# kocurvik/mdrp

Hardware: AMD Instinct MI355X
Metric: image-pairs/sec (2000 corrs, 10k RANSAC iters) (higher is better)
Workload: dtype f64

## Files before the change

### include/mdrp.h

```cpp
#ifndef MDRP_H
#define MDRP_H
#include <stddef.h>
#include <stdint.h>

#ifdef __cplusplus
extern "C" {
#endif

enum { MDRP_CALIB = 0, MDRP_SHARED_FOCAL = 1, MDRP_VARYING_FOCAL = 2,
       MDRP_RELPOSE_5PT = 3, MDRP_FUNDAMENTAL_7PT = 5,
       MDRP_SHARED_6PT = 4 };

enum {
    MDRP_OK = 0,
    MDRP_ERR_INVALID = 1,
    MDRP_ERR_HIP = 2,
    MDRP_ERR_NO_DEVICE = 3,
    MDRP_ERR_UNSUPPORTED = 4
};

enum {
    MDRP_MEM_HOST = 0,
    MDRP_MEM_DEVICE = 1
};

typedef struct {
    double q[4];
    double t[3];
    double scale, shift1, shift2;
    double f1, f2;
} mdrp_model;

typedef struct {
    uint64_t max_iterations;
    uint64_t min_iterations;
    double dyn_num_trials_mult;
    double success_prob;
    double max_reproj_error;
    double max_epipolar_error;
    uint64_t seed;
    int32_t monodepth_estimate_shift;
    float monodepth_weight_sampson;
    int32_t score_initial_model;
    int32_t progressive_sampling;
    uint64_t max_prosac_iterations;
    int32_t real_focal_check;
    int32_t reserved_;
} mdrp_ransac_opt;

typedef struct {
    uint64_t max_iterations;
    int32_t loss_type;
    double loss_scale;
    double gradient_tol;
    double step_tol;
    double initial_lambda;
    double min_lambda;
    double max_lambda;
} mdrp_bundle_opt;

typedef struct {
    int32_t model_id;
    int32_t pad_;
    double params[4];
} mdrp_camera;

typedef struct {
    mdrp_model model;
    uint64_t refinements, iterations, num_inliers;
    double inlier_ratio, model_score;
} mdrp_result;

typedef struct mdrp_handle mdrp_handle;

int mdrp_create_(int device, void *stream, mdrp_handle **out, int abi_version, int ransac_opt_bytes);
int mdrp_create_on_stream_(int device, void *stream, mdrp_handle **out, int abi_version, int ransac_opt_bytes);
#define mdrp_create(device, stream, out) mdrp_create_((device), (stream), (out), MDRP_ABI_VERSION, (int)sizeof(mdrp_ransac_opt))
#define mdrp_create_on_stream(device, stream, out) mdrp_create_on_stream_((device), (stream), (out), MDRP_ABI_VERSION, (int)sizeof(mdrp_ransac_opt))
void mdrp_destroy(mdrp_handle *h);
const char *mdrp_last_error(void);
const char *mdrp_version(void);
#define MDRP_ABI_VERSION 0x00000006
int mdrp_abi_version(void);
int mdrp_hip_build_version(void);
int mdrp_synchronize(mdrp_handle *h);


int mdrp_estimate_batch(mdrp_handle *h, int kind, int mem_space, const double *x1, const double *x2, const double *d1,
                        const double *d2, int batch, int n_max, const int32_t *n_per_pair, const mdrp_camera *cam1,
                        const mdrp_camera *cam2, const mdrp_ransac_opt *ropt, const mdrp_bundle_opt *bopt,
                        mdrp_result *out, uint8_t *inlier_mask);

int mdrp_estimate_batch_async(mdrp_handle *h, int kind, const double *x1_dev, const double *x2_dev, const double *d1_dev,
                              const double *d2_dev, int batch, int n_max, const int32_t *n_per_pair_host,
                              const mdrp_camera *cam1_host, const mdrp_camera *cam2_host, const mdrp_ransac_opt *ropt,
                              const mdrp_bundle_opt *bopt, uint8_t *inlier_mask_dev);
int mdrp_fetch_results(mdrp_handle *h, mdrp_result *out_host, int batch);
int mdrp_copy_results_device(mdrp_handle *h, void *dst_dev, int batch);

int mdrp_solver_batch(mdrp_handle *h, int solver, const double *x1h, const double *x2h, const double *d1,
                      const double *d2, int count, mdrp_model *out, int32_t *n_out);

int mdrp_classic_solver_batch(mdrp_handle *h, int kind, const double *x1h, const double *x2h, int count, mdrp_model *out,
                              int32_t *n_out);

int mdrp_score_models(mdrp_handle *h, int kind, int mem_space, const mdrp_model *models, int num_models,
                      const double *x1, const double *x2, int n, double sq_threshold, double *scores, int32_t *counts);

int mdrp_count_candidates(mdrp_handle *h, int kind, const mdrp_model *models, int num_models, const double *x1,
                          const double *x2, int n, double sq_threshold, int32_t *candidates);

int mdrp_bound_models(mdrp_handle *h, int kind, const mdrp_model *models, int num_models, const double *x1, const double *x2,
                      int n, double sq_threshold, double *score_lb, int32_t *count_ub);

#define MDRP_RETIRE_TWO_PHASE 1
#define MDRP_RETIRE_BOUND 2
#define MDRP_RETIRE_SWEEP_SCORE 0
#define MDRP_RETIRE_SWEEP_SPLIT 4
#define MDRP_RETIRE_SWEEP_WAVE 8
int mdrp_retire_models(mdrp_handle *h, int kind, const mdrp_model *models, int num_models, const double *x1, const double *x2,
                       int n, double sq_threshold, uint64_t rec_cnt, double rec_score, const uint64_t *cand_stat_in, int flags,
                       double *scores, int32_t *counts, int32_t *left_at, int32_t *info, uint64_t *cand_stat_out);

typedef struct {
    int32_t n, active;
    double sq_thr;
    uint64_t best_min_cnt;
    double best_min_score;
    uint64_t dyn_max_iter, iterations, refinements, num_inliers;
    double inlier_ratio, model_score;
    mdrp_model best;
} mdrp_replay_state;
typedef struct {
    uint32_t iter;
    int32_t k_ref;
    int32_t k_min;
    int32_t cnt_min;
    double score_min;
    int32_t cnt_ref;
    int32_t pad_;
} mdrp_replay_trigger;
typedef struct {
    int32_t mps, sample_sz, batch, n_chunks;
    uint64_t chunk_start;
    const int32_t *chunk_lens;
    const double *slot_score;
    const int32_t *slot_inl;
    const mdrp_model *models;
    const double *lo_score;
    const int32_t *lo_cnt;
    const mdrp_model *lo_models;
    const uint64_t *budgets;
    int32_t n_budgets, pad_;
    mdrp_replay_state *states;
    mdrp_replay_state *checkpoints;
    mdrp_replay_trigger *triggers;
    int32_t *n_triggers;
    uint64_t *scan_cnt;
    double *scan_score;
    int32_t *scan_inst;
    int32_t *lo_plan;
    int32_t *n_active;
    uint64_t *max_needed;
} mdrp_replay;
int mdrp_replay_slots(mdrp_handle *h, const mdrp_ransac_opt *ropt, mdrp_replay *io);

int mdrp_refine_models(mdrp_handle *h, int kind, mdrp_model *models, int count, const double *x1, const double *x2,
                       const double *d1, const double *d2, int n, double scale_reproj, double weight_sampson,
                       const mdrp_bundle_opt *opt, int estimate_shift, double *final_cost );

int mdrp_last_sweep_stats(mdrp_handle *h, double *sweep_ms, int64_t *launches, int64_t *evaluations);

typedef struct {
    double count_ms;
    int64_t count_launches;
    double sweep_ms;
    int64_t sweep_launches;
    int64_t evals_algorithmic;
    int64_t evals_mfma;
    int64_t evals_fp64;
    int64_t evals_bound;
    double lo_ms;
    int64_t lo_launches;
    double final_ms;
// ... 120 lines not shown
```

### mdrp_amd/_capi.py

```python
import ctypes as C
import os
import threading

import numpy as np

_HERE = os.path.dirname(os.path.abspath(__file__))
LIB_PATH = os.environ.get("MDRP_LIB") or os.path.join(_HERE, "libmdrp_hip.so")

CALIB, SHARED_FOCAL, VARYING_FOCAL = 0, 1, 2
RELPOSE_5PT, SHARED_6PT, FUNDAMENTAL_7PT = 3, 4, 5
MEM_HOST, MEM_DEVICE = 0, 1
SOLVER_P3P, SOLVER_SHIFT, SOLVER_SHARED, SOLVER_VARYING = 0, 1, 2, 3

EXPORTS = (
    "mdrp_create_", "mdrp_create_on_stream_", "mdrp_destroy", "mdrp_last_error", "mdrp_version", "mdrp_abi_version", "mdrp_hip_build_version", "mdrp_synchronize", "mdrp_estimate_batch",
    "mdrp_estimate_batch_async", "mdrp_fetch_results", "mdrp_copy_results_device", "mdrp_solver_batch", "mdrp_score_models", "mdrp_count_candidates", "mdrp_bound_models", "mdrp_refine_models",
    "mdrp_last_sweep_stats", "mdrp_last_stats", "mdrp_last_stats_sized", "mdrp_classic_solver_batch",
    "mdrp_gather_matches", "mdrp_estimate_matches_async",
    "mdrp_estimate_batch_budgets", "mdrp_estimate_batch_budgets_async", "mdrp_fetch_budget_results", "mdrp_copy_budget_results_device",
    "mdrp_refine_batch", "mdrp_refine_batch_async",
    "mdrp_gather_image_pairs", "mdrp_estimate_image_pairs_async",
    "mdrp_estimate_batch_prior", "mdrp_estimate_batch_prior_async",
    "mdrp_retire_models", "mdrp_replay_slots",
    "mdrp_estimate_batch_ranked", "mdrp_estimate_batch_ranked_async", "mdrp_prosac_samples", "mdrp_rank_scores",
    "mdrp_gather_matches_ranked", "mdrp_estimate_matches_ranked_async", "mdrp_gather_image_pairs_ranked", "mdrp_estimate_image_pairs_ranked_async",
)
RETIRE_TWO_PHASE, RETIRE_BOUND, RETIRE_SWEEP_SCORE, RETIRE_SWEEP_SPLIT, RETIRE_SWEEP_WAVE = 1, 2, 0, 4, 8
STAGE_LO, STAGE_INLIERS = 1, 2
MAX_BUDGETS = 16
F32, F64 = 0, 1
FILTERS = {"both_inf": 0, "finite": 1}


class Model(C.Structure):
    _fields_ = [("q", C.c_double * 4), ("t", C.c_double * 3), ("scale", C.c_double), ("shift1", C.c_double),
                ("shift2", C.c_double), ("f1", C.c_double), ("f2", C.c_double)]


class RansacOpt(C.Structure):
    _fields_ = [("max_iterations", C.c_uint64), ("min_iterations", C.c_uint64), ("dyn_num_trials_mult", C.c_double),
                ("success_prob", C.c_double), ("max_reproj_error", C.c_double), ("max_epipolar_error", C.c_double),
                ("seed", C.c_uint64), ("monodepth_estimate_shift", C.c_int32), ("monodepth_weight_sampson", C.c_float),
                ("score_initial_model", C.c_int32), ("progressive_sampling", C.c_int32), ("max_prosac_iterations", C.c_uint64),
                ("real_focal_check", C.c_int32), ("reserved_", C.c_int32)]


class BundleOpt(C.Structure):
    _fields_ = [("max_iterations", C.c_uint64), ("loss_type", C.c_int32), ("loss_scale", C.c_double),
                ("gradient_tol", C.c_double), ("step_tol", C.c_double), ("initial_lambda", C.c_double),
                ("min_lambda", C.c_double), ("max_lambda", C.c_double)]


class Camera(C.Structure):
    _fields_ = [("model_id", C.c_int32), ("pad_", C.c_int32), ("params", C.c_double * 4)]


class Stats(C.Structure):
    _fields_ = [("count_ms", C.c_double), ("count_launches", C.c_int64), ("sweep_ms", C.c_double), ("sweep_launches", C.c_int64),
                ("evals_algorithmic", C.c_int64), ("evals_mfma", C.c_int64), ("evals_fp64", C.c_int64), ("evals_bound", C.c_int64),
                ("lo_ms", C.c_double), ("lo_launches", C.c_int64), ("final_ms", C.c_double), ("final_launches", C.c_int64),
                ("bound_ms", C.c_double), ("bound_launches", C.c_int64), ("solve_ms", C.c_double), ("solve_launches", C.c_int64),
                ("lm_cost_evals", C.c_int64), ("lm_accum_evals", C.c_int64), ("final_cost_evals", C.c_int64), ("final_accum_evals", C.c_int64),
                ("fuse_gate_timeouts", C.c_int64), ("fuse_wait_timeouts", C.c_int64),
                ("first_chunk", C.c_int64)]


class Matches(C.Structure):
    _fields_ = [("kp1", C.c_void_p), ("kp2", C.c_void_p), ("kp_type", C.c_int32), ("k1", C.c_int32), ("k2", C.c_int32),
                ("matches", C.c_void_p), ("m_max", C.c_int32), ("depth1", C.c_void_p), ("depth2", C.c_void_p), ("depth_type", C.c_int32),
                ("h1", C.c_int32), ("w1", C.c_int32), ("h2", C.c_int32), ("w2", C.c_int32), ("center1", C.c_void_p), ("center2", C.c_void_p),
                ("filter", C.c_int32)]


class ImagePairs(C.Structure):
    _fields_ = [("kp", C.c_void_p), ("kp_type", C.c_int32), ("k_max", C.c_int32), ("kp_count", C.c_void_p), ("depth", C.c_void_p),
                ("depth_type", C.c_int32), ("h_max", C.c_int32), ("w_max", C.c_int32), ("size", C.c_void_p), ("center", C.c_void_p),
                ("n_images", C.c_int32), ("pairs", C.c_void_p), ("matches", C.c_void_p), ("m_max", C.c_int32), ("filter", C.c_int32)]


class Result(C.Structure):
    _fields_ = [("model", Model), ("refinements", C.c_uint64), ("iterations", C.c_uint64), ("num_inliers", C.c_uint64),
                ("inlier_ratio", C.c_double), ("model_score", C.c_double)]


MODEL_DTYPE = np.dtype([("q", "f8", 4), ("t", "f8", 3), ("scale", "f8"), ("shift1", "f8"), ("shift2", "f8"), ("f1", "f8"), ("f2", "f8")])
RESULT_DTYPE = np.dtype([("model", MODEL_DTYPE), ("refinements", "u8"), ("iterations", "u8"), ("num_inliers", "u8"),
                         ("inlier_ratio", "f8"), ("model_score", "f8")])
CAMERA_DTYPE = np.dtype([("model_id", "i4"), ("pad_", "i4"), ("params", "f8", 4)])
assert MODEL_DTYPE.itemsize == C.sizeof(Model) and RESULT_DTYPE.itemsize == C.sizeof(Result) and CAMERA_DTYPE.itemsize == C.sizeof(Camera)

REPLAY_STATE_DTYPE = np.dtype([("n", "i4"), ("active", "i4"), ("sq_thr", "f8"), ("best_min_cnt", "u8"), ("best_min_score", "f8"), ("dyn_max_iter", "u8"),
                               ("iterations", "u8"), ("refinements", "u8"), ("num_inliers", "u8"), ("inlier_ratio", "f8"), ("model_score", "f8"),
                               ("best", MODEL_DTYPE)])
REPLAY_TRIGGER_DTYPE = np.dtype([("iter", "u4"), ("k_ref", "i4"), ("k_min", "i4"), ("cnt_min", "i4"), ("score_min", "f8"), ("cnt_ref", "i4"), ("pad_", "i4")])


class Replay(C.Structure):
    _fields_ = [("mps", C.c_int32), ("sample_sz", C.c_int32), ("batch", C.c_int32), ("n_chunks", C.c_int32), ("chunk_start", C.c_uint64),
                ("chunk_lens", C.c_void_p), ("slot_score", C.c_void_p), ("slot_inl", C.c_void_p), ("models", C.c_void_p), ("lo_score", C.c_void_p),
                ("lo_cnt", C.c_void_p), ("lo_models", C.c_void_p), ("budgets", C.c_void_p), ("n_budgets", C.c_int32), ("pad_", C.c_int32),
# ... 12 lines not shown


def load_library():
    global _lib
    with _lib_lock:
        if _lib is not None:
            return _lib
        if not os.path.exists(LIB_PATH):
            raise MdrpError(f"{LIB_PATH} is not built (run __graft_entry__.build()); mdrp_amd has no CPU fallback")
        _ensure_hip_runtime()
        lib = C.CDLL(LIB_PATH)
        _check_hip_runtime_version(lib)
        vp, dp, ip = C.c_void_p, C.c_void_p, C.c_void_p
        lib.mdrp_last_error.restype = C.c_char_p
        lib.mdrp_version.restype = C.c_char_p
        abi = getattr(lib, "mdrp_abi_version", None)
        if abi is None or getattr(lib, "mdrp_create_", None) is None:
            raise MdrpError(f"{LIB_PATH} predates ABI {ABI_VERSION:#x} (no mdrp_abi_version / mdrp_create_): rebuild (mdrp_amd/build.py)")
        abi.restype = C.c_int
        if abi() != ABI_VERSION:
            raise MdrpError(f"{LIB_PATH} speaks ABI {abi():#x}, this binding {ABI_VERSION:#x}: rebuild (mdrp_amd/build.py)")
        lib.mdrp_create_.argtypes = [C.c_int, vp, C.POINTER(vp), C.c_int, C.c_int]
        lib.mdrp_create_on_stream_.argtypes = [C.c_int, vp, C.POINTER(vp), C.c_int, C.c_int]
        lib.mdrp_destroy.argtypes = [vp]
        lib.mdrp_destroy.restype = None
        lib.mdrp_synchronize.argtypes = [vp]
        lib.mdrp_estimate_batch.argtypes = [vp, C.c_int, C.c_int, dp, dp, dp, dp, C.c_int, C.c_int, ip, vp, vp,
                                            C.POINTER(RansacOpt), C.POINTER(BundleOpt), vp, vp]
        lib.mdrp_estimate_batch_async.argtypes = [vp, C.c_int, dp, dp, dp, dp, C.c_int, C.c_int, ip, vp, vp,
                                                  C.POINTER(RansacOpt), C.POINTER(BundleOpt), vp]
        lib.mdrp_fetch_results.argtypes = [vp, vp, C.c_int]
        lib.mdrp_copy_results_device.argtypes = [vp, vp, C.c_int]
        lib.mdrp_solver_batch.argtypes = [vp, C.c_int, dp, dp, dp, dp, C.c_int, vp, vp]
        lib.mdrp_score_models.argtypes = [vp, C.c_int, C.c_int, vp, C.c_int, dp, dp, C.c_int, C.c_double, vp, vp]
        lib.mdrp_count_candidates.argtypes = [vp, C.c_int, vp, C.c_int, dp, dp, C.c_int, C.c_double, vp]
        lib.mdrp_bound_models.argtypes = [vp, C.c_int, vp, C.c_int, dp, dp, C.c_int, C.c_double, vp, vp]
        lib.mdrp_refine_models.argtypes = [vp, C.c_int, vp, C.c_int, dp, dp, dp, dp, C.c_int, C.c_double, C.c_double,
                                           C.POINTER(BundleOpt), C.c_int, vp]
        lib.mdrp_last_sweep_stats.argtypes = [vp, C.POINTER(C.c_double), C.POINTER(C.c_int64), C.POINTER(C.c_int64)]
        lib.mdrp_last_stats.argtypes = [vp, C.POINTER(Stats)]
        lib.mdrp_last_stats_sized.argtypes = [vp, C.POINTER(Stats), C.c_size_t]
        lib.mdrp_classic_solver_batch.argtypes = [vp, C.c_int, dp, dp, C.c_int, vp, vp]
        lib.mdrp_gather_matches.argtypes = [vp, C.POINTER(Matches), C.c_int, dp, dp, dp, dp, ip, ip]
        lib.mdrp_estimate_matches_async.argtypes = [vp, C.c_int, C.POINTER(Matches), C.c_int, vp, vp, C.POINTER(RansacOpt), C.POINTER(BundleOpt), vp, ip]
        if hasattr(lib, "mdrp_estimate_batch_budgets"):
            lib.mdrp_estimate_batch_budgets.argtypes = [vp, C.c_int, C.c_int, dp, dp, dp, dp, C.c_int, C.c_int, ip, vp, vp,
                                                        C.POINTER(RansacOpt), C.POINTER(BundleOpt), vp, C.c_int, vp, vp]
            lib.mdrp_estimate_batch_budgets_async.argtypes = [vp, C.c_int, dp, dp, dp, dp, C.c_int, C.c_int, ip, vp, vp,
                                                              C.POINTER(RansacOpt), C.POINTER(BundleOpt), vp, C.c_int, vp]
            lib.mdrp_fetch_budget_results.argtypes = [vp, vp, C.c_int, C.c_int]
            lib.mdrp_copy_budget_results_device.argtypes = [vp, vp, C.c_int, C.c_int]
        if hasattr(lib, "mdrp_refine_batch"):
            lib.mdrp_refine_batch.argtypes = [vp, C.c_int, C.c_int, dp, dp, dp, dp, C.c_int, C.c_int, ip, vp, vp,
                                              C.POINTER(RansacOpt), C.POINTER(BundleOpt), vp, C.c_int, vp, vp, dp, ip]
            lib.mdrp_refine_batch_async.argtypes = [vp, C.c_int, dp, dp, dp, dp, C.c_int, C.c_int, ip, vp, vp,
                                                    C.POINTER(RansacOpt), C.POINTER(BundleOpt), vp, C.c_int, vp, dp, ip]
        if hasattr(lib, "mdrp_gather_image_pairs"):
            lib.mdrp_gather_image_pairs.argtypes = [vp, C.POINTER(ImagePairs), C.c_int, dp, dp, dp, dp, ip, ip]
            lib.mdrp_estimate_image_pairs_async.argtypes = [vp, C.c_int, C.POINTER(ImagePairs), C.c_int, vp, vp, C.POINTER(RansacOpt), C.POINTER(BundleOpt), vp, ip]
        if hasattr(lib, "mdrp_estimate_batch_ranked"):
            lib.mdrp_estimate_batch_ranked.argtypes = [vp, C.c_int, C.c_int, dp, dp, dp, dp, dp, C.c_int, C.c_int, ip, vp, vp,
                                                       C.POINTER(RansacOpt), C.POINTER(BundleOpt), vp, vp]
            lib.mdrp_estimate_batch_ranked_async.argtypes = [vp, C.c_int, dp, dp, dp, dp, dp, C.c_int, C.c_int, ip, vp, vp,
                                                             C.POINTER(RansacOpt), C.POINTER(BundleOpt), vp]
            lib.mdrp_prosac_samples.argtypes = [vp, C.c_uint64, C.c_int, C.c_uint64, ip, C.c_int, vp]
            lib.mdrp_rank_scores.argtypes = [vp, C.c_int, vp, C.c_int, C.c_int, ip, vp]
        if hasattr(lib, "mdrp_gather_matches_ranked"):
            lib.mdrp_gather_matches_ranked.argtypes = [vp, C.POINTER(Matches), vp, C.c_int, C.c_int, dp, dp, dp, dp, ip, ip]
            lib.mdrp_estimate_matches_ranked_async.argtypes = [vp, C.c_int, C.POINTER(Matches), vp, C.c_int, C.c_int, vp, vp, C.POINTER(RansacOpt),
                                                               C.POINTER(BundleOpt), vp, ip]
            lib.mdrp_gather_image_pairs_ranked.argtypes = [vp, C.POINTER(ImagePairs), vp, C.c_int, C.c_int, dp, dp, dp, dp, ip, ip]
            lib.mdrp_estimate_image_pairs_ranked_async.argtypes = [vp, C.c_int, C.POINTER(ImagePairs), vp, C.c_int, C.c_int, vp, vp, C.POINTER(RansacOpt),
                                                                   C.POINTER(BundleOpt), vp, ip]
        if hasattr(lib, "mdrp_estimate_batch_prior"):
            lib.mdrp_estimate_batch_prior.argtypes = [vp, C.c_int, C.c_int, dp, dp, dp, dp, C.c_int, C.c_int, ip, vp, vp,
                                                      C.POINTER(RansacOpt), C.POINTER(BundleOpt), vp, vp, vp]
            lib.mdrp_estimate_batch_prior_async.argtypes = [vp, C.c_int, dp, dp, dp, dp, C.c_int, C.c_int, ip, vp, vp,
                                                            C.POINTER(RansacOpt), C.POINTER(BundleOpt), vp, vp]
        if hasattr(lib, "mdrp_retire_models"):
            lib.mdrp_retire_models.argtypes = [vp, C.c_int, vp, C.c_int, dp, dp, C.c_int, C.c_double, C.c_uint64, C.c_double, vp, C.c_int,
                                               vp, vp, vp, vp, vp]
        if hasattr(lib, "mdrp_replay_slots"):
            lib.mdrp_replay_slots.argtypes = [vp, C.POINTER(RansacOpt), C.POINTER(Replay)]
        _lib = lib
        return lib


ABI_VERSION = 0x00000006
ERR_UNSUPPORTED = 4


def _check(lib, rc):
    if rc == ERR_UNSUPPORTED:
        raise NotImplementedError(f"mdrp: {lib.mdrp_last_error().decode(errors='replace')} (DESIGN.md 9)")
    if rc != 0:
        raise MdrpError(f"mdrp error {rc}: {lib.mdrp_last_error().decode(errors='replace')}")


def _ptr(a):
    return None if a is None else C.c_void_p(a.ctypes.data)


def ransac_opt_from_dict(d=None):
    d = d or {}
    return RansacOpt(int(d.get("max_iterations", 100000)), int(d.get("min_iterations", 1000)),
                     float(d.get("dyn_num_trials_mult", 3.0)), float(d.get("success_prob", 0.9999)),
                     float(d.get("max_reproj_error", 12.0)), float(d.get("max_epipolar_error", 1.0)),
                     int(d.get("seed", 0)), int(bool(d.get("monodepth_estimate_shift", False))),
                     float(d.get("monodepth_weight_sampson", 1.0)), int(bool(d.get("score_initial_model", False))),
                     int(bool(d.get("progressive_sampling", False))), int(d.get("max_prosac_iterations", 100000)),
                     int(bool(d.get("real_focal_check", False))), 0)


LOSS_TYPES = {"TRIVIAL": 0, "TRUNCATED": 1, "HUBER": 2, "CAUCHY": 3, "TRUNCATED_CAUCHY": 4, "TRUNCATED_LE_ZACH": 5}


def bundle_opt_from_dict(d=None):
    d = d or {}
    lt = d.get("loss_type", "CAUCHY")
    if isinstance(lt, str):
        if lt.upper() not in LOSS_TYPES:
            raise ValueError(f"unknown loss_type {lt!r}")
        lt = LOSS_TYPES[lt.upper()]
    return BundleOpt(int(d.get("max_iterations", 100)), int(lt), float(d.get("loss_scale", 1.0)),
                     float(d.get("gradient_tol", 1e-10)), float(d.get("step_tol", 1e-8)), float(d.get("initial_lambda", 1e-3)),
                     float(d.get("min_lambda", 1e-10)), float(d.get("max_lambda", 1e10)))


def budget_list(budgets, ransac_opt=None):
    try:
        ks = [int(k) for k in budgets]
        exact = all(k == b for k, b in zip(ks, budgets))
    except (TypeError, ValueError):
        raise ValueError("budgets must be a sequence of integers") from None
    if not ks:
        raise ValueError("budgets: an empty list")
    if not exact:
        raise ValueError("budgets must be integers")
    if len(ks) > MAX_BUDGETS:
        raise ValueError(f"budgets: more than {MAX_BUDGETS}")
    if ks[0] < 1 or any(b <= a for a, b in zip(ks, ks[1:])):
        raise ValueError("budgets must be >= 1 and strictly increasing")
    ro = dict(ransac_opt or {})
    if "max_iterations" in ro and int(ro["max_iterations"]) != ks[-1]:
        raise ValueError(f"ransac_opt['max_iterations'] = {ro['max_iterations']} differs from the last budget {ks[-1]}")
    ro["max_iterations"] = ks[-1]
    return np.asarray(ks, dtype=np.uint64), ro


def library_version():
    return load_library().mdrp_version().decode()


def library_source_hash():
    v = library_version()
    return v.split("MDRP_SRC_HASH=", 1)[1][:16] if "MDRP_SRC_HASH=" in v else None


_hip_runtime = None
hip_versions = None


def _check_hip_runtime_version(lib):
    import warnings
    try:
        lib.mdrp_hip_build_version.restype = C.c_int
        built = int(lib.mdrp_hip_build_version())
        v = C.c_int(0)
        rt = _hip_runtime.hipRuntimeGetVersion
        rt.argtypes = [C.POINTER(C.c_int)]
        if rt(C.byref(v)) != 0:
            return
    except (AttributeError, OSError):
        return
    have = int(v.value)
    if have // 10_000_000 != built // 10_000_000:
        raise MdrpError(f"libmdrp_hip.so was built against HIP {built // 10_000_000}.{built // 100_000 % 100} but the process's HIP runtime "
                        f"({getattr(_hip_runtime, '_name', '?')}) is {have // 10_000_000}.{have // 100_000 % 100}: set MDRP_HIP_RUNTIME to a "
                        "matching libamdhip64.so or rebuild (mdrp_amd/build.py)")
    global hip_versions
    hip_versions = {"built": built, "runtime": have}
    if have // 100_000 != built // 100_000 and os.environ.get("MDRP_DEBUG"):
        warnings.warn(f"mdrp: HIP runtime {have // 10_000_000}.{have // 100_000 % 100} in this process, library built against "
                      f"{built // 10_000_000}.{built // 100_000 % 100} (same major: continuing)", RuntimeWarning, stacklevel=3)


def _ensure_hip_runtime():
    global _hip_runtime
    if _hip_runtime is not None:
        return _hip_runtime
    import sys
    cands = []
    if os.environ.get("MDRP_HIP_RUNTIME"):
        cands.append(os.environ["MDRP_HIP_RUNTIME"])
    try:
        torch = sys.modules.get("torch")
        if torch is not None:
            tdir = os.path.dirname(torch.__file__)
        else:
            import importlib.util
            spec = importlib.util.find_spec("torch")
            tdir = list(spec.submodule_search_locations)[0] if spec is not None and spec.submodule_search_locations else None
        if tdir and os.path.exists(os.path.join(tdir, "lib", "libamdhip64.so")):
            cands.append(os.path.join(tdir, "lib", "libamdhip64.so"))
    except Exception:
        pass
    import glob
    rocm = os.environ.get("ROCM_PATH", "/opt/rocm")
    def _soname_version(path):
        tail = os.path.basename(path).split(".so.", 1)[-1]
        return tuple(int(x) for x in tail.split(".") if x.isdigit())
    cands += sorted(glob.glob(os.path.join(rocm, "lib", "libamdhip64.so.*")), key=_soname_version, reverse=True) + ["libamdhip64.so", os.path.join(rocm, "lib", "libamdhip64.so")]
    errs = []
    for c in cands:
        try:
            _hip_runtime = C.CDLL(c, mode=C.RTLD_GLOBAL)
            return _hip_runtime
        except OSError as e:
            errs.append(f"{c}: {e}")
    raise MdrpError("no HIP runtime (libamdhip64) could be loaded: " + "; ".join(errs))


class Handle:

    def __init__(self, device=0, stream=None):
        self._lib = load_library()
        h = C.c_void_p()
        if stream is None:
            _check(self._lib, self._lib.mdrp_create_(int(device), None, C.byref(h), ABI_VERSION, C.sizeof(RansacOpt)))
        else:
# ... 475 lines not shown
```

### mdrp_amd/build.py

```python
import hashlib
import os
import re
import shutil
import subprocess

HERE = os.path.dirname(os.path.abspath(__file__))
SRC = os.path.join(HERE, "csrc", "mdrp_capi.hip")
SRC_TU = os.path.join(HERE, "csrc", "mdrp_tu.hip")
TU_GROUPS = (1, 2, 3, 4, 5)
DEPS = [SRC, SRC_TU, os.path.join(HERE, "csrc", "mdrp_kernels.h"), os.path.join(HERE, "csrc", "mdrp_math.h"),
        os.path.join(HERE, "csrc", "mdrp_classic.h"), os.path.join(HERE, "csrc", "mdrp_classic_math.h"),
        os.path.join(HERE, "csrc", "mdrp_logtab.h"), os.path.join(HERE, "csrc", "mdrp_instances.h"),
        os.path.join(HERE, "csrc", "mdrp_frontend.h"), os.path.join(HERE, "csrc", "mdrp_schedule.h"),
        os.path.join(HERE, "csrc", "mdrp_from_model.h"), os.path.join(HERE, "csrc", "mdrp_prior.h"), os.path.join(HERE, "csrc", "mdrp_prosac.h"),
        os.path.join(HERE, "..", "include", "mdrp.h")]
OUT = os.path.join(HERE, "libmdrp_hip.so")
_MARK = b"MDRP_SRC_HASH="
FLAGS = ["-O3", "-std=c++17", "--offload-arch=gfx950", "-fPIC", "-shared", "-ffp-contract=fast", "-no-hip-rt"]


def hipcc():
    for c in (shutil.which("hipcc"), "/opt/rocm/bin/hipcc"):
        if c and os.path.exists(c):
            return c
    raise RuntimeError("hipcc not found")


def source_hash():
    h = hashlib.sha256()
    h.update(" ".join(FLAGS).encode())
    for d in DEPS:
        h.update(os.path.basename(d).encode() + b"\0")
        with open(d, "rb") as f:
            h.update(f.read())
    return h.hexdigest()[:16]


def built_hash(path=OUT):
    try:
        with open(path, "rb") as f:
            m = re.search(_MARK + rb"([0-9a-f]{16})", f.read())
        return m.group(1).decode() if m else None
    except OSError:
        return None


def up_to_date():
    return built_hash() == source_hash()


def build(force=False, verbose=False, defines=(), out=OUT, extra_flags=(), single=None):
    if not force and not defines and not extra_flags and out == OUT and up_to_date():
        return out
    if single is None:
        single = bool(defines) or bool(extra_flags)
    common = [*FLAGS, *extra_flags, f'-DMDRP_SRC_HASH="{source_hash()}"', *[f"-D{d}" for d in defines]]
    if verbose:
        common.insert(0, "-Rpass-analysis=kernel-resource-usage")
    if single:
        subprocess.check_call([hipcc(), *common, SRC, "-o", out + ".tmp"])
        os.replace(out + ".tmp", out)
        return out
    import tempfile
    from concurrent.futures import ThreadPoolExecutor
    cflags = [f for f in common if f != "-shared"]
    with tempfile.TemporaryDirectory(prefix="mdrp_build_") as tmp:
        jobs = [([hipcc(), *cflags, "-DMDRP_SPLIT_TU", "-c", SRC, "-o", os.path.join(tmp, "capi.o")], os.path.join(tmp, "capi.o"))]
        for g in TU_GROUPS:
            obj = os.path.join(tmp, f"tu{g}.o")
            jobs.append(([hipcc(), *cflags, f"-DMDRP_TU={g}", "-c", SRC_TU, "-o", obj], obj))

        def run(job):
            r = subprocess.run(job[0], capture_output=True, text=True)
            return job, r
        with ThreadPoolExecutor(max_workers=len(jobs)) as pool:
            results = list(pool.map(run, jobs))
        for (cmd, obj), r in results:
            if verbose or r.returncode != 0:
                import sys
                sys.stderr.write(r.stderr)
            if r.returncode != 0:
                raise subprocess.CalledProcessError(r.returncode, cmd, r.stdout, r.stderr)
        subprocess.check_call([hipcc(), "--offload-arch=gfx950", "-shared", "-fPIC", "-no-hip-rt", *[o for _, o in jobs], "-o", out + ".tmp"])
    os.replace(out + ".tmp", out)
    return out


if __name__ == "__main__":
    print(build(force=True, verbose=True))
```

### mdrp_amd/csrc/mdrp_capi.hip

```cpp
#include "../../include/mdrp.h"
#include "mdrp_kernels.h"
#include "mdrp_classic.h"
#include "mdrp_frontend.h"
#include "mdrp_schedule.h"
#include "mdrp_from_model.h"
#include "mdrp_prior.h"
#include "mdrp_prosac.h"
#ifdef MDRP_SPLIT_TU
#define MDRP_INST extern
#include "mdrp_instances.h"
namespace mdrp {
MDRP_INSTANCES_FINAL_64
MDRP_INSTANCES_FINAL_256
MDRP_INSTANCES_CLASSIC
MDRP_INSTANCES_FROM_MODEL
MDRP_INSTANCES_PRIOR
}
#endif

#include <algorithm>
#include <cmath>
#include <cstdio>
#include <cstdlib>
#include <cstddef>
// ... 29 lines not shown
struct DevBuf {
    void *p = nullptr;
    size_t cap = 0;
    DevBuf() = default;
    DevBuf(const DevBuf &) = delete;
    DevBuf &operator=(const DevBuf &) = delete;
    ~DevBuf() { release(); }
    int ensure(size_t bytes) {
        if (bytes <= cap) return MDRP_OK;
        if (p) { (void)hipFree(p); p = nullptr; cap = 0; }
        size_t want = bytes + bytes / 8 + 256;
        hipError_t e = hipMalloc(&p, want);
        if (e != hipSuccess) { g_err = std::string("hipMalloc failed: ") + hipGetErrorString(e); p = nullptr; return MDRP_ERR_HIP; }
        cap = want;
        return MDRP_OK;
    }
    void release() { if (p) (void)hipFree(p); p = nullptr; cap = 0; }
    template <typename T> T *as() const { return reinterpret_cast<T *>(p); }
};

template <typename T, auto Destroy> struct Owned {
    T v = nullptr;
    Owned() = default;
    Owned(Owned &&o) noexcept : v(o.v) { o.v = nullptr; }
    Owned(const Owned &) = delete;
    Owned &operator=(const Owned &) = delete;
    ~Owned() { reset(); }
    void reset() { if (v) (void)Destroy(v); v = nullptr; }
    operator T() const { return v; }
    T operator->() const { return v; }
};
using Stream = Owned<hipStream_t, hipStreamDestroy>;
using Event = Owned<hipEvent_t, hipEventDestroy>;
template <typename T> using Pinned = Owned<T *, hipHostFree>;

struct Progress {
    int32_t n_active, pad_;
    unsigned long long max_needed;
    unsigned long long evals;
    unsigned long long evals_mfma;
    unsigned long long evals_sweep;
    unsigned long long evals_bound;
    int32_t wish_sum, wish_pairs;
};
struct Counters {
    int32_t unused_[2];
    Progress progress;
    int32_t lo_head[16];
    int32_t xcd_head[8 * LO_XCD_STRIDE];
};
static_assert(offsetof(Counters, progress) == 2 * sizeof(int32_t) && offsetof(Counters, lo_head) == 16 * sizeof(int32_t) &&
              offsetof(Counters, xcd_head) == 32 * sizeof(int32_t) && sizeof(Counters) == 640, "counter block layout");
static_assert(offsetof(Progress, evals_mfma) == offsetof(Progress, evals) + sizeof(unsigned long long), "k_count adds to stats[0] and stats[1]");
static_assert(offsetof(Progress, wish_pairs) == offsetof(Progress, wish_sum) + sizeof(int32_t), "RunParams::inl_stat is [2]");
constexpr size_t LM_STATS_BYTES = 6 * sizeof(unsigned long long);

struct DeviceGuard {
    int prev = -1;
    bool ok = true;
    explicit DeviceGuard(int device) {
        if (hipGetDevice(&prev) != hipSuccess) prev = -1;
        if (prev != device) ok = hipSetDevice(device) == hipSuccess;
    }
    ~DeviceGuard() {
        int cur = -1;
        if (prev >= 0 && hipGetDevice(&cur) == hipSuccess && cur != prev) (void)hipSetDevice(prev);
    }
};

}

struct mdrp_handle {
    std::mutex mu;
    int device = 0;
    hipStream_t stream = nullptr;
    Stream own_stream;
    Stream aux_stream;
    Stream aux_stream2;
    Stream copy_stream;
    Event ev_copied, ev_prepped, ev_solved6;
    DevBuf fuse;
    Event ev_lo, ev_tables, ev_sampled[2], ev_solved[sched::NC_MAX], ev_scanned[sched::NC_MAX];
    int num_cu = 256;
    DevBuf pts, dep, st;
    DevBuf params;
    Pinned<unsigned char> params_host;
    size_t params_host_cap = 0;
    DevBuf models, slot_score, slot_inl, triggers, work_pair, counters, results, mask, plan;
    DevBuf samples[2], tags[2], model_count[2];
    DevBuf tags_sorted[2];
    DevBuf tags_v, surv_count;
    DevBuf cand_stat;
    DevBuf und_count;
    DevBuf rfrag;
    DevBuf cplan;
    DevBuf surv2_count;
    DevBuf lo_mask;
    DevBuf red5;
    DevBuf lm_stats;
    Pinned<unsigned long long> lm_stats_host;
    int64_t fuse_gate_timeouts = 0, fuse_wait_timeouts = 0;
    int64_t first_chunk = 0;
    double seen_wish[3] = {-1.0, -1.0, -1.0};
    Pinned<int32_t> wish_host; Event ev_wish;
    int wish_kind = -1;
    bool fuse_disabled = false;
    int fuse_retry_in = 0;
    int fuse_backoff = 64;
    DevBuf ckpt, ck_list, bresults, bmask;
    int last_budgets = 0;
    DevBuf in_x1, in_x2, in_d1, in_d2;
    DevBuf fm_models, fm_init;
    DevBuf pr_x1, pr_x2, pr_d1, pr_d2, pr_order, pr_mask, pr_scores, pr_nper, pr_tab;
    DevBuf fe_key;
    DevBuf fe_x1, fe_x2, fe_d1, fe_d2, fe_slot, fe_n;
    Pinned<int32_t> fe_n_host;
    size_t fe_n_host_cap = 0;
    DevBuf unit_a, unit_b, unit_c, unit_d, unit_e, unit_f;
    Pinned<Progress> progress_host;
    std::vector<std::pair<Event, Event>> ev_pool;
    std::vector<int> ev_what;
    size_t ev_used = 0;
    double sweep_ms = 0.0, count_ms = 0.0;
    double kind_ms[6] = {0, 0, 0, 0, 0, 0};
    int64_t kind_launches[6] = {0, 0, 0, 0, 0, 0};
    int64_t lm_cost_evals = 0, lm_accum_evals = 0, fin_cost_evals = 0, fin_accum_evals = 0;
    int64_t count_launches = 0;
    int64_t sweep_launches = 0, sweep_evals = 0, mfma_evals = 0, fp64_evals = 0, bound_evals = 0;
    int last_batch = 0;
};

namespace {

#define MDRP_LM_DISPATCH_T(KERNEL, T, kind, shift, grid, smem, stream, ...)                                          \
    do {                                                                                                             \
        if ((kind) == 0 && (shift)) hipLaunchKernelGGL((KERNEL<0, true, T>), grid, dim3(T), smem, stream, __VA_ARGS__);  \
        else if ((kind) == 0) hipLaunchKernelGGL((KERNEL<0, false, T>), grid, dim3(T), smem, stream, __VA_ARGS__);       \
        else if ((kind) == 1) hipLaunchKernelGGL((KERNEL<1, false, T>), grid, dim3(T), smem, stream, __VA_ARGS__);       \
        else hipLaunchKernelGGL((KERNEL<2, false, T>), grid, dim3(T), smem, stream, __VA_ARGS__);                        \
    } while (0)
#define MDRP_LM_DISPATCH(KERNEL, threads, kind, shift, grid, smem, stream, ...)                                      \
    do {                                                                                                             \
        if ((threads) == 64) MDRP_LM_DISPATCH_T(KERNEL, 64, kind, shift, grid, smem, stream, __VA_ARGS__);           \
        else MDRP_LM_DISPATCH_T(KERNEL, 256, kind, shift, grid, smem, stream, __VA_ARGS__);                          \
    } while (0)

#define MDRP_FINAL_DISPATCH_L(T, FL, kind, shift, grid, smem, stream, ...)                                                  \
    do {                                                                                                                   \
        if ((kind) == 0 && (shift)) hipLaunchKernelGGL((k_final<0, true, T, FL>), grid, dim3(T), smem, stream, __VA_ARGS__);  \
        else if ((kind) == 0) hipLaunchKernelGGL((k_final<0, false, T, FL>), grid, dim3(T), smem, stream, __VA_ARGS__);       \
        else if ((kind) == 1) hipLaunchKernelGGL((k_final<1, false, T, FL>), grid, dim3(T), smem, stream, __VA_ARGS__);       \
        else hipLaunchKernelGGL((k_final<2, false, T, FL>), grid, dim3(T), smem, stream, __VA_ARGS__);                        \
    } while (0)
#define MDRP_FINAL_DISPATCH_T(T, floss, kind, shift, grid, smem, stream, ...)                                               \
    do {                                                                                                                   \
        switch (floss) {                                                                                                   \
        case 1: MDRP_FINAL_DISPATCH_L(T, 1, kind, shift, grid, smem, stream, __VA_ARGS__); break;                          \
        case 2: MDRP_FINAL_DISPATCH_L(T, 2, kind, shift, grid, smem, stream, __VA_ARGS__); break;                          \
        case 3: MDRP_FINAL_DISPATCH_L(T, 3, kind, shift, grid, smem, stream, __VA_ARGS__); break;                          \
        case 4: MDRP_FINAL_DISPATCH_L(T, 4, kind, shift, grid, smem, stream, __VA_ARGS__); break;                          \
        case 5: MDRP_FINAL_DISPATCH_L(T, 5, kind, shift, grid, smem, stream, __VA_ARGS__); break;                          \
        default: MDRP_FINAL_DISPATCH_L(T, 0, kind, shift, grid, smem, stream, __VA_ARGS__); break;  \
        }                                                                                                                  \
    } while (0)
#define MDRP_FINAL_DISPATCH(threads, floss, kind, shift, grid, smem, stream, ...)                                           \
    do {                                                                                                                   \
// ... 105 lines not shown
}
constexpr int HOST_SLICE_PAIRS = 256;

struct PassIn {
    int kind;
    const double *x1, *x2, *d1, *d2;
    int batch, n_max;
    const int32_t *n_host;
    const mdrp_camera *cam1, *cam2;
    const mdrp_ransac_opt *ro;
    const mdrp_bundle_opt *bo;
    int chunk_cap;
    uint8_t *mask_dev;
    ResultDev *results_dev;
    const HostSrc *host;
    int batch_call;
    const BudgetOut *bud;
    const Model *priors;
    const uint64_t *prosac;
};

struct ProsacTab { uint64_t *k; const uint64_t *off; const uint32_t *sub; };
void launch_samples_prosac(hipStream_t st, int threads, int n_tables, const int32_t *d_table_n, uint64_t *d_table_state, const ProsacTab &tab,
                           uint64_t max_prosac, int len, uint32_t *smp) {
    hipLaunchKernelGGL(k_samples_prosac, dim3(n_tables), dim3(threads), 0, st, n_tables, d_table_n, d_table_state, tab.k, tab.off, tab.sub,
                       prosac::prosac_samples(max_prosac), len, smp);
}
int prosac_tables(mdrp_handle *h, hipStream_t s, const int32_t *tab_n, int n_tables, uint64_t max_prosac, uint64_t count, ProsacTab &tab) {
    std::vector<uint64_t> head(2 * (size_t)n_tables + 1, 0);
    std::vector<uint32_t> sub;
    for (int t = 0; t < n_tables; ++t) {
        const std::vector<uint32_t> one = prosac::subset_schedule((uint64_t)std::max(tab_n[t], 0), max_prosac, count, true);
        head[n_tables + t] = sub.size();
        sub.insert(sub.end(), one.begin(), one.end());
    }
    head[2 * (size_t)n_tables] = sub.size();
    const size_t hb = sizeof(uint64_t) * head.size(), sb = sizeof(uint32_t) * sub.size();
    if (int rc = h->pr_tab.ensure(hb + sb + 16)) return rc;
    unsigned char *d = h->pr_tab.as<unsigned char>();
    HIPCHK(hipMemcpyAsync(d, head.data(), hb, hipMemcpyHostToDevice, s));
    if (sb) HIPCHK(hipMemcpyAsync(d + hb, sub.data(), sb, hipMemcpyHostToDevice, s));
    tab.k = reinterpret_cast<uint64_t *>(d); tab.off = tab.k + n_tables; tab.sub = reinterpret_cast<const uint32_t *>(d + hb);
    return MDRP_OK;
}

int launch_scan(hipStream_t s, int mps, int pairs, const RunParams &r, PairState *st, const double *slot_score, const int32_t *slot_inl, Trigger *trig,
                int trig_cap, const int32_t *model_count, unsigned long long *scan_stats) {
#define MDRP_SCAN(M, I)                                                                                                                            \
    do {                                                                                                                                           \
        hipLaunchKernelGGL((k_scan<M, I>), dim3(pairs), dim3(64), 0, s, r, st, slot_score, slot_inl, trig, trig_cap, model_count, scan_stats);      \
        return 10 * M + I;                                                                                                                         \
    } while (0)
    if (mps == 16) MDRP_SCAN(16, 1);
    if (mps == 12) MDRP_SCAN(12, 1);
    if (r.chunk_len >= 1024) MDRP_SCAN(4, 4);
    MDRP_SCAN(4, 1);
#undef MDRP_SCAN
}

struct ChunkView {
    int c, p0, pc;
    bool first_of_run;
    RunParams r;
    PairState *st;
    double *pts, *dep, *slot_score;
    Model *models;
    int32_t *slot_inl, *model_count, *surv1, *surv2, *und_count;
    uint32_t *samples, *tags, *tags_sorted, *tags_sorted_other, *tags_v;
    unsigned long long *cand_stat;
    uint4 *rfrag;
    Trigger *trig;
};
struct Survivors { const uint32_t *tags; const int32_t *count; };

struct Pass : PassIn {
    mdrp_handle *const h;
    const hipStream_t s;
    const int est_shift;
    const bool classic;
    const int mps, ssz;
    const bool lo_overlap = env_int("MDRP_LO_OVERLAP", 1) != 0;
    const bool use_bound = env_int("MDRP_BOUND", 1) != 0;
    const bool score_split = env_int("MDRP_SCORE_SPLIT", 1) != 0;
    const int lo_threads = env_int("MDRP_LO_THREADS", sched::lo_lanes(batch_call, n_max));
    const int final_threads = env_int("MDRP_FINAL_THREADS", sched::final_lanes(batch_call));
    const int samp_threads = env_int("MDRP_SAMPLE_THREADS", ssz == 3 ? SAMP_THREADS : (ssz == 5 ? 512 : 256));
    const int lo_blocks = h->num_cu * (lo_threads == 64 ? 8 : 2);
    const int mask_index = lm_mask_index_on(n_max);
    const int clm_list_stride = lm_list_stride(n_max);
    const size_t clm_list_bytes = (size_t)2 * clm_list_stride * sizeof(uint16_t);
    const bool fuse_env = !bud && env_int("MDRP_FUSE_TAIL", ((kind == MDRP_CALIB && est_shift) || h->fuse_disabled) ? 0 : 1) != 0;
    const int n_bud = bud ? bud->n : 0;
    const int trig_cap = chunk_cap;
    const size_t groups_max = ((size_t)n_max + 15) / 16;

    std::vector<int32_t> table_of, tab_n;
    int n_tables = 0;
    uint64_t certain = 0;
    sched::Lead lead;
    PassScratch sz;
    RunParams rp;
    unsigned char *pd = nullptr;
    uint64_t *d_table_state = nullptr;
    CamDev *d_cams1 = nullptr, *d_cams2 = nullptr;
    int32_t *d_table_n = nullptr, *d_table_of = nullptr, *d_nper = nullptr;
    Counters *cnt = nullptr;
    uint64_t it0 = 0;
    sched::Layout lay;
    bool piped = false, fuse_tail = false, presampled[2] = {false, false};
    hipStream_t aux = nullptr, aux2 = nullptr;
    int32_t *fz_ctl = nullptr, *fz_done = nullptr, *fz_fin = nullptr, *fz_ready = nullptr;
    bool final_done = false;
    ProsacTab ptab{nullptr, nullptr, nullptr};

    Pass(mdrp_handle *h_, const PassIn &in)
        : PassIn(in), h(h_), s(h_->stream), est_shift((kind == MDRP_CALIB && ro->monodepth_estimate_shift) ? 1 : 0), classic(kind >= MDRP_RELPOSE_5PT),
          mps(sched::model_slots(kind)), ssz(sched::sample_size(kind)) {}

    int plan_and_allocate() {
        sched::group_tables(n_host, batch, table_of, tab_n);
        n_tables = (int)tab_n.size();
        certain = sched::certain_iterations(ro->max_iterations, ro->min_iterations);
        const bool chunks_set = sched::parse_chunks(getenv("MDRP_CHUNKS"), lead);
        if (h->wish_kind >= 0 && hipEventQuery(h->ev_wish) == hipSuccess) {
            if (h->wish_host[1] > 0) h->seen_wish[h->wish_kind] = (double)h->wish_host[0] / (double)h->wish_host[1];
            h->wish_kind = -1;
        }
        if (!chunks_set) lead = sched::default_lead(kind, certain, kind <= MDRP_VARYING_FOCAL ? h->seen_wish[kind] : -1.0);
        sz = pass_scratch(h, kind, batch, n_max, n_tables, chunk_cap, lead.first(), n_bud);
        for (const auto &b : sz.bufs) {
            if (int rc = b.first->ensure(b.second)) return rc;
            if (b.first == &h->params && h->params_host_cap < sz.params) {
                h->params_host.reset(); h->params_host_cap = 0;
                HIPCHK(hipHostMalloc((void **)&h->params_host.v, sz.params + sz.params / 2, hipHostMallocDefault));
                h->params_host_cap = sz.params + sz.params / 2;
            }
        }
        pd = h->params.as<unsigned char>();
        d_table_state = reinterpret_cast<uint64_t *>(pd);
        d_cams1 = reinterpret_cast<CamDev *>(pd + sz.off_cam1); d_cams2 = reinterpret_cast<CamDev *>(pd + sz.off_cam2);
        d_table_n = reinterpret_cast<int32_t *>(pd + sz.off_tn); d_table_of = reinterpret_cast<int32_t *>(pd + sz.off_tof);
        d_nper = reinterpret_cast<int32_t *>(pd + sz.off_nper);
        cnt = h->counters.as<Counters>();
        return MDRP_OK;
    }

    int upload_params() {
        unsigned char *ph = h->params_host;
        const std::vector<uint64_t> tab_state(n_tables, ro->seed);
        std::memcpy(ph, tab_state.data(), sizeof(uint64_t) * n_tables);
        const bool cams = kind == MDRP_CALIB || kind == MDRP_RELPOSE_5PT || kind == MDRP_SHARED_6PT;
        if (cams) { std::memcpy(ph + sz.off_cam1, cam1, sizeof(CamDev) * batch); std::memcpy(ph + sz.off_cam2, cam2 ? cam2 : cam1, sizeof(CamDev) * batch); }
        else std::memset(ph + sz.off_cam1, 0, 2 * sizeof(CamDev) * (size_t)batch);
        std::memcpy(ph + sz.off_tn, tab_n.data(), sizeof(int32_t) * n_tables);
        std::memcpy(ph + sz.off_tof, table_of.data(), sizeof(int32_t) * batch);
        std::memcpy(ph + sz.off_nper, n_host, sizeof(int32_t) * batch);
        if (bud) std::memcpy(ph + sz.off_bud, bud->budgets, sizeof(uint64_t) * n_bud);
        HIPCHK(hipMemcpyAsync(pd, ph, sz.params, hipMemcpyHostToDevice, s));
        if (prosac) { if (int rc = prosac_tables(h, s, tab_n.data(), n_tables, *prosac, ro->max_iterations, ptab)) return rc; }

        std::memset(&rp, 0, sizeof rp);
        rp.kind = kind; rp.solver = solver_for(kind, est_shift); rp.est_shift = est_shift;
        rp.score_initial = ro->score_initial_model ? 1 : 0;
        rp.batch = batch; rp.n_max = n_max;
        rp.max_iterations = ro->max_iterations; rp.min_iterations = ro->min_iterations;
        rp.dyn_mult = ro->dyn_num_trials_mult; rp.log_prob_missing = std::log(1.0 - ro->success_prob);
// ... 1 lines not shown
        rp.final_max_it = (int)std::min<uint64_t>(bo->max_iterations, 1u << 30); rp.final_loss = bo->loss_type;
        rp.grad_tol = bo->gradient_tol; rp.step_tol = bo->step_tol; rp.lambda0 = bo->initial_lambda;
        rp.lambda_min = bo->min_lambda; rp.lambda_max = bo->max_lambda;
        rp.chunk_len = chunk_cap; rp.chunk_off = 0; rp.slot_stride = chunk_cap * mps; rp.super_len = chunk_cap; rp.chunk_start = 0;
        rp.mps = mps; rp.sample_sz = ssz;
        return MDRP_OK;
    }

    void prep(int p0, int pc, hipStream_t st_) {
        const size_t o2 = (size_t)2 * p0 * n_max, o1 = (size_t)p0 * n_max;
        double *pts_p = h->pts.as<double>() + o1 * PT_STRIDE;
        uint4 *rfrag_p = h->rfrag.as<uint4>() + (size_t)p0 * groups_max * 64;
        if (classic)
            hipLaunchKernelGGL(kc_prep, dim3(pc), dim3(256), 0, st_, rp, x1 + o2, x2 + o2, d_nper + p0, d_table_of + p0, d_cams1 + p0, d_cams2 + p0,
                               ro->max_epipolar_error, bo->loss_scale, pts_p, h->st.as<PairState>() + p0, rfrag_p);
        else
            hipLaunchKernelGGL(k_prep, dim3(pc), dim3(256), 0, st_, rp, x1 + o2, x2 + o2, d1 + o1, d2 + o1, d_nper + p0, d_table_of + p0, d_cams1 + p0, d_cams2 + p0,
                               ro->max_epipolar_error, ro->max_reproj_error, bo->loss_scale, pts_p, h->dep.as<double>() + 2 * o1, h->st.as<PairState>() + p0, rfrag_p);
    }

    void prior() {
#define MDRP_PRIOR_LAUNCH(K, S)                                                                                                                  \
    hipLaunchKernelGGL((k_prior<K, S>), dim3(batch), dim3(PRIOR_THREADS), lm_list_bytes(n_max), s, rp, h->st.as<PairState>(),                     \
                       (const double *)h->pts.as<double>(), (const double *)h->dep.as<double>(), priors, lm_list_stride(n_max),                  \
                       h->lm_stats.as<unsigned long long>())
        if (kind == MDRP_CALIB && est_shift) MDRP_PRIOR_LAUNCH(0, true);
        else if (kind == MDRP_CALIB) MDRP_PRIOR_LAUNCH(0, false);
        else if (kind == MDRP_SHARED_FOCAL) MDRP_PRIOR_LAUNCH(1, false);
        else MDRP_PRIOR_LAUNCH(2, false);
#undef MDRP_PRIOR_LAUNCH
    }

    int begin_super_chunk(uint64_t max_needed) {
        lay = sched::super_chunk_layout(it0, certain, chunk_cap, lead, max_needed, ro->max_iterations);
        if (it0 == 0) h->first_chunk = (int64_t)lay.lens[0];
        rp.chunk_start = it0; rp.super_len = (int)lay.super_len;
        HIPCHK(hipMemsetAsync(h->counters.p, 0, sizeof(Counters), s));
        if (it0 == 0) HIPCHK(hipMemsetAsync(h->cand_stat.p, 0, sizeof(unsigned long long) * 2 * batch, s));
        piped = lay.n_chunks > 1 && lo_overlap;
        fuse_tail = fuse_env && piped && it0 + lay.super_len >= ro->max_iterations;
        if (fuse_tail) {
            if (int rc = h->fuse.ensure(sz.fuse)) return rc;
            fz_ctl = h->fuse.as<int32_t>(); fz_done = fz_ctl + 16; fz_fin = fz_done + batch; fz_ready = fz_fin + batch;
        }
        aux = piped ? h->aux_stream : s; aux2 = piped ? h->aux_stream2 : s;
        presampled[0] = presampled[1] = false;
        return MDRP_OK;
    }

    void samples(hipStream_t st_, int len_, uint32_t *smp_) {
        if (prosac) launch_samples_prosac(st_, samp_threads, n_tables, d_table_n, d_table_state, ptab, *prosac, len_, smp_);
        else if (ssz == 6) hipLaunchKernelGGL(kc_samples<6>, dim3(n_tables), dim3(samp_threads), 0, st_, n_tables, d_table_n, d_table_state, len_, smp_);
        else if (ssz == 5) hipLaunchKernelGGL(kc_samples<5>, dim3(n_tables), dim3(samp_threads), 0, st_, n_tables, d_table_n, d_table_state, len_, smp_);
        else if (ssz == 7) hipLaunchKernelGGL(kc_samples<7>, dim3(n_tables), dim3(samp_threads), 0, st_, n_tables, d_table_n, d_table_state, len_, smp_);
        else hipLaunchKernelGGL(k_samples, dim3(n_tables), dim3(samp_threads), 0, st_, n_tables, d_table_n, d_table_state, len_, smp_);
    }
    int presample() {
        HIPCHK(hipStreamWaitEvent(aux2, h->ev_tables, 0));
        for (int c = 0; c < 2 && c < lay.n_chunks; ++c) {
            samples(aux2, (int)lay.lens[c], h->samples[c & 1].as<uint32_t>());
            HIPCHK(hipEventRecord(h->ev_sampled[c], aux2));
            presampled[c] = true;
        }
        return MDRP_OK;
    }

    ChunkView view(int c, int p0, int pc) const {
        ChunkView v;
        const bool odd = c & 1;
        const size_t so = (size_t)p0 * rp.slot_stride, o1 = (size_t)p0 * n_max, q = (size_t)p0;
        v.c = c; v.p0 = p0; v.pc = pc; v.first_of_run = it0 == 0 && c == 0;
        v.r = rp; v.r.chunk_len = (int)lay.lens[c]; v.r.chunk_off = lay.offs[c]; v.r.batch = pc;
        v.st = h->st.as<PairState>() + q; v.pts = h->pts.as<double>() + o1 * PT_STRIDE; v.dep = classic ? nullptr : h->dep.as<double>() + o1 * 2;
        v.models = h->models.as<Model>() + so; v.slot_score = h->slot_score.as<double>() + so; v.slot_inl = h->slot_inl.as<int32_t>() + so;
        v.samples = h->samples[odd].as<uint32_t>(); v.tags = h->tags[odd].as<uint32_t>() + so; v.tags_v = h->tags_v.as<uint32_t>() + so;
        v.tags_sorted = h->tags_sorted[odd].as<uint32_t>() + so; v.tags_sorted_other = h->tags_sorted[!odd].as<uint32_t>() + so;
        v.model_count = h->model_count[odd].as<int32_t>() + 2 * q; v.und_count = h->und_count.as<int32_t>() + 2 * q;
        v.surv1 = h->surv_count.as<int32_t>() + q; v.surv2 = h->surv2_count.as<int32_t>() + q;
        v.cand_stat = h->cand_stat.as<unsigned long long>() + 2 * q;
        v.rfrag = h->rfrag.as<uint4>() + q * groups_max * 64; v.trig = h->triggers.as<Trigger>() + q * trig_cap;
        return v;
    }

    int solve(const ChunkView &v, hipStream_t st_) {
        const RunParams &r = v.r;
        const int pc = v.pc;
        HIPCHK(hipMemsetAsync(v.model_count, 0, sizeof(int32_t) * 2 * pc, st_));
        if (v.c < 2 && presampled[v.c]) HIPCHK(hipStreamWaitEvent(st_, h->ev_sampled[v.c], 0));
        else samples(st_, r.chunk_len, v.samples);
        hipEvent_t v0, v1;
        if (int rc = get_events(h, &v0, &v1, 5)) return rc;
        HIPCHK(hipEventRecord(v0, st_));
        struct Stop { hipEvent_t e; hipStream_t s; ~Stop() { (void)hipEventRecord(e, s); } } stop_{v1, st_};
        if (classic) {
            const dim3 sgrid((r.chunk_len + 63) / 64, pc);
            if (kind == MDRP_SHARED_6PT)
                hipLaunchKernelGGL(kc_solve<CLASSIC_SHARED>, sgrid, dim3(64), 0, st_, r, v.st, v.samples, v.pts, v.models, v.slot_inl, v.tags, v.model_count);
            else if (kind == MDRP_RELPOSE_5PT) {
                const bool first_region = v.c == 0 && lay.n_chunks > 1;
                if (first_region && (size_t)sgrid.x > sz.red5_first_blocks) { g_err = "5-point first chunk longer than its Reduce5 region"; return MDRP_ERR_INVALID; }
                double *red5 = h->red5.as<double>() + ((first_region ? (size_t)batch * sz.red5_blocks : 0) + (size_t)v.p0 * sgrid.x) * RED5_STRIDE * 64;
                hipLaunchKernelGGL(kc_solve5_null, sgrid, dim3(64), SOLVE5N_LDS_BYTES, st_, r, v.st, v.samples, v.pts, red5);
                hipLaunchKernelGGL(kc_solve5_reduce, sgrid, dim3(64), SOLVE5_LDS_BYTES, st_, r, v.st, red5);
                hipLaunchKernelGGL(kc_solve5_roots, sgrid, dim3(64), SOLVE5B_LDS_BYTES, st_, r, v.st, v.samples, v.pts, red5, v.models, v.slot_inl, v.tags, v.model_count);
            }
            else
                hipLaunchKernelGGL(kc_solve<CLASSIC_FUND>, sgrid, dim3(64), SOLVE7_LDS_BYTES, st_, r, v.st, v.samples, v.pts, v.models, v.slot_inl, v.tags, v.model_count);
            return MDRP_OK;
        }
#define MDRP_SOLVE_LAUNCH(S)                                                                                                   \
    hipLaunchKernelGGL(k_solve<S>, dim3((r.chunk_len + solve_threads(S) - 1) / solve_threads(S), pc), dim3(solve_threads(S)), 0, st_, r, v.st, v.samples, v.pts, v.dep, v.models, v.slot_inl, v.tags, v.model_count, 0, r.chunk_len)
        switch (r.solver) {
        case SOLVER_P3P: MDRP_SOLVE_LAUNCH(SOLVER_P3P); break;
        case SOLVER_SHIFT: MDRP_SOLVE_LAUNCH(SOLVER_SHIFT); break;
        case SOLVER_SHARED: MDRP_SOLVE_LAUNCH(SOLVER_SHARED); break;
        default: MDRP_SOLVE_LAUNCH(SOLVER_VARYING); break;
        }
#undef MDRP_SOLVE_LAUNCH
        return MDRP_OK;
    }

    int count(const ChunkView &v) {
        unsigned long long *cstats = &cnt->progress.evals;
        hipEvent_t c0, c1;
        if (int rc = get_events(h, &c0, &c1, 1)) return rc;
        const bool two_phase = !v.first_of_run;
        uint32_t *tags_u = v.tags_sorted;
        int32_t *und_part = reinterpret_cast<int32_t *>(v.tags_sorted_other), *cplan = h->cplan.as<int32_t>();
        hipLaunchKernelGGL(k_count_plan, dim3(1), dim3(PLAN_THREADS), 0, s, v.pc, v.st, v.model_count, 2, CNT_WG_MODELS, cplan,
                           v.surv1, (const int32_t *)nullptr, two_phase ? v.und_count : (int32_t *)nullptr);
        const dim3 cgrid((unsigned)v.pc * (unsigned)((v.r.chunk_len * mps + CNT_WG_MODELS - 1) / CNT_WG_MODELS));
        HIPCHK(hipEventRecord(c0, s));
        MDRP_SWEEP_DISPATCH(k_count, kind, cgrid, dim3(CNT_THREADS), 0, s, v.r, v.st, v.rfrag, v.models,
                            v.tags, v.model_count, cplan, v.tags_v, v.surv1, cstats, (int32_t *)nullptr, (const int32_t *)nullptr,
                            1, tags_u, und_part, v.und_count, (const int32_t *)nullptr, v.cand_stat);
        if (two_phase) {
            hipLaunchKernelGGL(k_count_plan, dim3(1), dim3(PLAN_THREADS), 0, s, v.pc, v.st, v.und_count, 2, CNT_WG_MODELS, cplan,
                               (int32_t *)nullptr, (const int32_t *)nullptr, (int32_t *)nullptr);
            MDRP_SWEEP_DISPATCH(k_count, kind, cgrid, dim3(CNT_THREADS), 0, s, v.r, v.st, v.rfrag, v.models,
                                tags_u, v.und_count, cplan, v.tags_v, v.surv1, cstats, (int32_t *)nullptr, (const int32_t *)nullptr,
                                2, (uint32_t *)nullptr, (int32_t *)nullptr, (int32_t *)nullptr, und_part, v.cand_stat);
            h->count_launches++;
        }
        HIPCHK(hipEventRecord(c1, s));
        h->count_launches++;
        return MDRP_OK;
    }

    int bound(const ChunkView &v, Survivors &sv) {
        sv = Survivors{v.tags_v, v.surv1};
        if (!(use_bound && batch_call > 16 && !v.first_of_run)) return MDRP_OK;
        hipLaunchKernelGGL(k_count_plan, dim3(1), dim3(PLAN_THREADS), 0, s, v.pc, v.st, v.surv1, 1, BND_THREADS, h->cplan.as<int32_t>(), v.surv2, (const int32_t *)nullptr);
        const dim3 bgrid((unsigned)v.pc * (unsigned)((v.r.chunk_len * mps + BND_THREADS - 1) / BND_THREADS));
        unsigned long long *bstats = &cnt->progress.evals_bound;
        hipEvent_t b0, b1;
        if (int rc = get_events(h, &b0, &b1, 4)) return rc;
        HIPCHK(hipEventRecord(b0, s));
        MDRP_SWEEP_DISPATCH(k_bound, kind, bgrid, dim3(BND_THREADS), 0, s, v.r, v.st, v.pts, v.models, v.tags_v, v.surv1, h->cplan.as<int32_t>(), v.tags, v.surv2, bstats);
        HIPCHK(hipEventRecord(b1, s));
        sv = Survivors{v.tags, v.surv2};
        return MDRP_OK;
    }

    int score(const ChunkView &v, const Survivors &sv, hipEvent_t e0, hipEvent_t e1) {
        const bool wave = batch_call <= SCORE_WAVE_MAX_PAIRS, split = !wave && score_split && !v.first_of_run;
        const int models = v.r.chunk_len * mps;
        int32_t *plan = h->plan.as<int32_t>(), *totals = plan + 2 * (size_t)batch + 2;
        if (wave) hipLaunchKernelGGL(k_count_plan, dim3(1), dim3(PLAN_THREADS), 0, s, v.pc, v.st, sv.count, 1, SCW_THREADS / 64, plan, (int32_t *)nullptr, (const int32_t *)nullptr, (int32_t *)nullptr);
        hipLaunchKernelGGL(k_sort_tags, dim3(v.pc), dim3(256), 0, s, v.r, v.st, v.model_count, sv.count, sv.tags, v.tags_sorted);
        if (!wave) hipLaunchKernelGGL(k_plan, dim3(1), dim3(PLAN_THREADS), 0, s, v.pc, v.model_count, plan, totals, split ? SPLIT_HYP : SCORE_THREADS);
        HIPCHK(hipEventRecord(e0, s));
        const long long capped = (long long)h->num_cu * 32;
        if (wave) {
            const long long ub = (long long)v.pc * ((models + SCW_THREADS / 64 - 1) / (SCW_THREADS / 64));
            MDRP_SWEEP_DISPATCH(k_score_w, kind, dim3((unsigned)std::min(ub, capped)), dim3(SCW_THREADS), 0, s, v.r, v.st, v.pts, v.models, v.tags_sorted, v.model_count,
                                v.slot_score, v.slot_inl, plan);
        } else if (split) {
            const long long ub = (long long)v.pc * ((models + SPLIT_HYP - 1) / SPLIT_HYP + 1);
            MDRP_SWEEP_DISPATCH(k_score_split, kind, dim3((unsigned)std::min(ub, capped)), dim3(SPLIT_THREADS), 0, s, v.r, v.st, v.pts, v.models, v.tags_sorted, v.model_count,
                                v.slot_score, v.slot_inl, plan, totals);
        } else {
            const dim3 grid((unsigned)v.pc * (unsigned)((models + SCORE_THREADS - 1) / SCORE_THREADS));
            MDRP_SWEEP_DISPATCH(k_score, kind, grid, dim3(SCORE_THREADS), SCORE_TILE_BYTES, s, v.r, v.st, v.pts, v.models, v.tags_sorted, v.model_count,
                                v.slot_score, v.slot_inl, plan, totals);
        }
        HIPCHK(hipEventRecord(e1, s));
        h->sweep_launches++;
        return MDRP_OK;
    }

    void scan(const ChunkView &v) {
        (void)launch_scan(s, mps, v.pc, v.r, v.st, v.slot_score, v.slot_inl, v.trig, trig_cap, v.model_count, &cnt->progress.evals_sweep);
    }

    int sweep(const ChunkView &v) {
        hipEvent_t e0, e1;
        Survivors sv;
        int rc;
        if ((rc = get_events(h, &e0, &e1, 0)) || (rc = count(v)) || (rc = bound(v, sv)) || (rc = score(v, sv, e0, e1))) return rc;
        scan(v);
        return MDRP_OK;
    }

    int first_chunk_of(int q0, int qc) {
        const ChunkView v = view(0, q0, qc);
        int rc;
        if (kind != MDRP_SHARED_6PT) { if ((rc = solve(v, s))) return rc; }
        else {
            if ((rc = solve(v, aux))) return rc;
            HIPCHK(hipEventRecord(h->ev_solved6, aux));
            HIPCHK(hipStreamWaitEvent(s, h->ev_solved6, 0));
        }
        return sweep(v);
    }
    int host_front(bool &solved1, int &swept0) {
        int rc;
        const bool sliced = piped && lay.n_chunks >= 2 && batch >= 2 * HOST_SLICE_PAIRS;
        const int sl = sliced ? HOST_SLICE_PAIRS : batch;
        for (int p0 = 0; p0 < batch; p0 += sl) {
            const int pc = std::min(sl, batch - p0);
            const size_t o2 = (size_t)2 * p0 * n_max, o1 = (size_t)p0 * n_max, n2 = sizeof(double) * 2 * (size_t)pc * n_max, n1 = sizeof(double) * (size_t)pc * n_max;
            hipStream_t cs = sliced ? h->copy_stream : s;
            HIPCHK(hipMemcpyAsync(const_cast<double *>(x1) + o2, host->x1 + o2, n2, hipMemcpyHostToDevice, cs));
            HIPCHK(hipMemcpyAsync(const_cast<double *>(x2) + o2, host->x2 + o2, n2, hipMemcpyHostToDevice, cs));
            if (host->d1 && host->d2) {
                HIPCHK(hipMemcpyAsync(const_cast<double *>(d1) + o1, host->d1 + o1, n1, hipMemcpyHostToDevice, cs));
                HIPCHK(hipMemcpyAsync(const_cast<double *>(d2) + o1, host->d2 + o1, n1, hipMemcpyHostToDevice, cs));
            }
            if (!sliced) { prep(p0, pc, s); break; }
            HIPCHK(hipEventRecord(h->ev_copied, cs)); HIPCHK(hipStreamWaitEvent(aux, h->ev_copied, 0));
            if (p0 == 0) HIPCHK(hipStreamWaitEvent(aux, h->ev_tables, 0));
            prep(p0, pc, aux);
            HIPCHK(hipEventRecord(h->ev_prepped, aux));
            if ((rc = solve(view(1, p0, pc), aux))) return rc;
            const bool last = p0 + sl >= batch, last_but_one = !last && p0 + 2 * sl >= batch;
            if (last_but_one || last) HIPCHK(hipStreamWaitEvent(s, h->ev_prepped, 0));
            if (last_but_one) { swept0 = p0 + pc; if ((rc = first_chunk_of(0, swept0))) return rc; }
            if (last) { if ((rc = first_chunk_of(swept0, batch - swept0))) return rc; swept0 = batch; }
        }
        if (sliced) { HIPCHK(hipEventRecord(h->ev_solved[1], aux)); solved1 = true; }
        return MDRP_OK;
    }

    int lo(int c) {
        int32_t *lo_plan = h->work_pair.as<int32_t>();
        hipLaunchKernelGGL(k_lo_plan, dim3(1), dim3(PLAN_THREADS), 0, s, batch, h->st.as<PairState>(), (const int32_t *)nullptr, lo_plan);
        if (fuse_tail) {
            HIPCHK(hipMemsetAsync(fz_ctl, 0, 64 + 2 * sizeof(int32_t) * (size_t)batch, s));
            HIPCHK(hipMemsetAsync(fz_ready, 0xFF, sizeof(int32_t) * (size_t)batch, s));
        }
        if (piped) { HIPCHK(hipEventRecord(h->ev_scanned[c], s)); HIPCHK(hipStreamWaitEvent(aux2, h->ev_scanned[c], 0)); }
        const FuseTail fz = fuse_tail ? FuseTail{fz_done, fz_ready, fz_ctl, h->st.as<PairState>()} : FuseTail{nullptr, nullptr, nullptr, nullptr};
        unsigned long long *lm_stats = h->lm_stats.as<unsigned long long>();
        int32_t *xheads = cnt->xcd_head;
        hipEvent_t l0, l1;
        if (int rc = get_events(h, &l0, &l1, 2)) return rc;
        HIPCHK(hipEventRecord(l0, aux2));
        if (classic)
            MDRP_CLASSIC_LM_DISPATCH(kc_lo, lo_threads, kind, dim3(lo_blocks), clm_list_bytes, aux2, rp, h->st.as<PairState>(), h->pts.as<double>(),
                                     h->models.as<Model>(), h->triggers.as<Trigger>(), trig_cap, lo_plan, cnt->lo_head, xheads,
                                     h->lo_mask.as<uint8_t>(), clm_list_stride, fz);
        else
            MDRP_LM_DISPATCH(k_lo, lo_threads, kind, est_shift, dim3(lo_blocks), lm_list_bytes(n_max), aux2, rp,
                             h->st.as<PairState>(), h->pts.as<double>(), h->dep.as<double>(), h->models.as<Model>(), h->triggers.as<Trigger>(),
                             trig_cap, lo_plan, cnt->lo_head, xheads, lm_list_stride(n_max), lm_stats, fz);
        HIPCHK(hipEventRecord(l1, aux2));
        return MDRP_OK;
    }

    void final_of(const RunParams &rf, int problems, PairState *st_f, uint8_t *mask_f, ResultDev *results_f, const int32_t *ready, int32_t *fin_done,
                  unsigned long long ticks, unsigned long long *timeouts) {
        if (classic)
            MDRP_CLASSIC_LM_DISPATCH(kc_final, final_threads, kind, dim3(problems), clm_list_bytes, s, rf, st_f, h->pts.as<double>(), mask_f, results_f,
                                     ready, fin_done, ticks, timeouts, clm_list_stride);
        else
            MDRP_FINAL_DISPATCH(final_threads, rf.final_loss, kind, est_shift, dim3(problems), (mask_index ? lm_final_list_bytes(n_max) : lm_list_bytes(n_max)), s, rf,
                                st_f, h->pts.as<double>(), h->dep.as<double>(), mask_f, results_f, lm_list_stride(n_max), mask_index,
                                h->lm_stats.as<unsigned long long>() + 2, ready, fin_done, ticks, timeouts);
    }
    void final_pairs(const int32_t *ready, int32_t *fin_done, unsigned long long ticks, unsigned long long *timeouts) {
        final_of(rp, batch, h->st.as<PairState>(), mask_dev, results_dev, ready, fin_done, ticks, timeouts);
    }
// ... 193 lines not shown
int finish_timing(mdrp_handle *h) {
    if (h->lm_stats.p) HIPCHK(hipMemcpyAsync(h->lm_stats_host, h->lm_stats.p, LM_STATS_BYTES, hipMemcpyDeviceToHost, h->stream));
    HIPCHK(hipStreamSynchronize(h->stream));
    h->lm_cost_evals = (int64_t)h->lm_stats_host[0]; h->lm_accum_evals = (int64_t)h->lm_stats_host[1];
    h->fin_cost_evals = (int64_t)h->lm_stats_host[2]; h->fin_accum_evals = (int64_t)h->lm_stats_host[3];
    h->fuse_gate_timeouts = (int64_t)h->lm_stats_host[4]; h->fuse_wait_timeouts = (int64_t)h->lm_stats_host[5];
    if (!(h->fuse_gate_timeouts || h->fuse_wait_timeouts) && !h->fuse_disabled) h->fuse_backoff = 64;
    if ((h->fuse_gate_timeouts || h->fuse_wait_timeouts) && !h->fuse_disabled) {
        h->fuse_disabled = true;
        h->fuse_retry_in = h->fuse_backoff;
        h->fuse_backoff = std::min(h->fuse_backoff * 2, 16384);
        if (!getenv("MDRP_QUIET"))
            fprintf(stderr, "[mdrp] fused tail: %lld gate / %lld final-refinement waits timed out (kernels of two streams did not overlap: "
                            "profiler or serialised dispatch?); this handle runs unfused for its next %d calls\n",
                    (long long)h->fuse_gate_timeouts, (long long)h->fuse_wait_timeouts, h->fuse_retry_in);
    }
    for (int k = 0; k < 6; ++k) { h->kind_ms[k] = 0; h->kind_launches[k] = 0; }
    for (size_t i = 0; i < h->ev_used; ++i) {
        float t = 0;
        HIPCHK(hipEventElapsedTime(&t, h->ev_pool[i].first, h->ev_pool[i].second));
        const int k = std::min(std::max(h->ev_what[i], 0), 5);
        h->kind_ms[k] += t; h->kind_launches[k]++;
    }
    h->sweep_ms = h->kind_ms[0]; h->count_ms = h->kind_ms[1];
    return MDRP_OK;
}

}

#define MDRP_ENTER(h)                                                                      \
    std::lock_guard<std::mutex> lock_((h)->mu);                                            \
    DeviceGuard guard_((h)->device);                                                       \
    if (!guard_.ok) { g_err = "hipSetDevice failed"; return MDRP_ERR_HIP; }

#ifndef MDRP_SRC_HASH
#define MDRP_SRC_HASH "unknown"
#endif

static int create_handle(int device, hipStream_t stream, bool own_stream, mdrp_handle **out);

extern "C" {

const char *mdrp_last_error(void) { return g_err.c_str(); }
int mdrp_abi_version(void) { return MDRP_ABI_VERSION; }
const char *mdrp_version(void) { return "mdrp-hip 0.6 (gfx950) MDRP_SRC_HASH=" MDRP_SRC_HASH; }

int mdrp_hip_build_version(void) { return HIP_VERSION; }

static int check_host_abi(int abi_version, int ransac_opt_bytes) {
    if (abi_version == MDRP_ABI_VERSION && ransac_opt_bytes == (int)sizeof(mdrp_ransac_opt)) return MDRP_OK;
    char buf[256];
    snprintf(buf, sizeof buf, "host was compiled against ABI %#x (mdrp_ransac_opt %d bytes), this library speaks %#x (%d bytes): recompile the host against include/mdrp.h",
             abi_version, ransac_opt_bytes, MDRP_ABI_VERSION, (int)sizeof(mdrp_ransac_opt));
    g_err = buf;
    return MDRP_ERR_INVALID;
}
int mdrp_create_(int device, void *stream, mdrp_handle **out, int abi_version, int ransac_opt_bytes) {
    if (int rc = check_host_abi(abi_version, ransac_opt_bytes)) return rc;
    return create_handle(device, (hipStream_t)stream, stream == nullptr, out);
}
int mdrp_create_on_stream_(int device, void *stream, mdrp_handle **out, int abi_version, int ransac_opt_bytes) {
    if (int rc = check_host_abi(abi_version, ransac_opt_bytes)) return rc;
    return create_handle(device, (hipStream_t)stream, false, out);
}

}

static int create_handle(int device, hipStream_t stream, bool own_stream, mdrp_handle **out) {
    if (!out) return MDRP_ERR_INVALID;
    int ndev = 0;
    if (hipGetDeviceCount(&ndev) != hipSuccess || ndev <= 0 || device < 0 || device >= ndev) {
        g_err = "no usable HIP device";
        return MDRP_ERR_NO_DEVICE;
    }
    DeviceGuard guard_(device);
    if (!guard_.ok) { g_err = "hipSetDevice failed"; return MDRP_ERR_HIP; }
    std::unique_ptr<mdrp_handle> h(new mdrp_handle());
    h->device = device;
    if (own_stream) HIPCHK(hipStreamCreateWithFlags(&h->own_stream.v, hipStreamNonBlocking));
    h->stream = own_stream ? h->own_stream.v : stream;
    hipDeviceProp_t prop;
    HIPCHK(hipGetDeviceProperties(&prop, device));
    h->num_cu = prop.multiProcessorCount > 0 ? prop.multiProcessorCount : 256;
    HIPCHK(hipHostMalloc((void **)&h->progress_host.v, sizeof(Progress), hipHostMallocDefault));
    HIPCHK(hipHostMalloc((void **)&h->lm_stats_host.v, LM_STATS_BYTES, hipHostMallocDefault));
    HIPCHK(hipHostMalloc((void **)&h->wish_host.v, 2 * sizeof(int32_t), hipHostMallocDefault));
    HIPCHK(hipEventCreateWithFlags(&h->ev_wish.v, hipEventDisableTiming));
    std::memset(h->lm_stats_host, 0, LM_STATS_BYTES);
    {
        int prio_lo = 0, prio_hi = 0;
        (void)hipDeviceGetStreamPriorityRange(&prio_lo, &prio_hi);
        HIPCHK(hipStreamCreateWithPriority(&h->aux_stream.v, hipStreamNonBlocking, prio_hi));
        HIPCHK(hipStreamCreateWithPriority(&h->aux_stream2.v, hipStreamNonBlocking, prio_hi));
    }
    HIPCHK(hipStreamCreateWithFlags(&h->copy_stream.v, hipStreamNonBlocking));
    for (Event *e : {&h->ev_copied, &h->ev_prepped, &h->ev_solved6, &h->ev_lo, &h->ev_tables, &h->ev_sampled[0], &h->ev_sampled[1]})
        HIPCHK(hipEventCreateWithFlags(&e->v, hipEventDisableTiming));
    for (int i = 0; i < sched::NC_MAX; ++i) {
        HIPCHK(hipEventCreateWithFlags(&h->ev_solved[i].v, hipEventDisableTiming));
        HIPCHK(hipEventCreateWithFlags(&h->ev_scanned[i].v, hipEventDisableTiming));
    }
    const int tile_bytes = (int)SCORE_TILE_BYTES;
    HIPCHK(hipFuncSetAttribute(reinterpret_cast<const void *>(k_score<true>), hipFuncAttributeMaxDynamicSharedMemorySize, tile_bytes));
    HIPCHK(hipFuncSetAttribute(reinterpret_cast<const void *>(k_score<false>), hipFuncAttributeMaxDynamicSharedMemorySize, tile_bytes));
    HIPCHK(hipFuncSetAttribute(reinterpret_cast<const void *>(k_score<false, true>), hipFuncAttributeMaxDynamicSharedMemorySize, tile_bytes));
    HIPCHK(hipFuncSetAttribute(reinterpret_cast<const void *>(kc_solve5_reduce), hipFuncAttributeMaxDynamicSharedMemorySize, (int)SOLVE5_LDS_BYTES));
    HIPCHK(hipFuncSetAttribute(reinterpret_cast<const void *>(kc_solver_unit<CLASSIC_RELPOSE>), hipFuncAttributeMaxDynamicSharedMemorySize, (int)SOLVE5_LDS_BYTES));
    *out = h.release();
    return MDRP_OK;
}

static int upload_iota(hipStream_t s, void *tags, int count) {
    std::vector<uint32_t> iota(count);
    for (int i = 0; i < count; ++i) iota[i] = (uint32_t)i;
    HIPCHK(hipMemcpyAsync(tags, iota.data(), sizeof(uint32_t) * count, hipMemcpyHostToDevice, s));
    return MDRP_OK;
}
static int stage_unit_pair(mdrp_handle *h, const double *x1, const double *x2, int n, double sq_threshold, uint64_t rec_cnt = 0,
                           double rec_score = DBL_MAX) {
    hipStream_t s = h->stream;
    PairState ps;
    std::memset(&ps, 0, sizeof ps);
    ps.n = n; ps.active = 1; ps.sq_thr = sq_threshold; ps.eps = std::sqrt(sq_threshold);
    ps.best_min_cnt = rec_cnt; ps.best_min_score = rec_score < DBL_MAX ? rec_score : DBL_MAX;
    HIPCHK(hipMemcpyAsync(h->st.p, &ps, sizeof ps, hipMemcpyHostToDevice, s));
    hipLaunchKernelGGL(k_pack_unit, dim3((n + 255) / 256 + 1), dim3(256), 0, s, n, x1, x2, (const double *)nullptr,
                       (const double *)nullptr, h->pts.as<double>(), (double *)nullptr);
    hipLaunchKernelGGL(k_box_unit, dim3(1), dim3(256), 0, s, n, h->pts.as<double>(), h->st.as<PairState>());
    return MDRP_OK;
}

static LmOpt lm_opt(const mdrp_bundle_opt *opt) {
    LmOpt o;
    o.max_it = (int)std::min<uint64_t>(opt->max_iterations, 1u << 30); o.loss = opt->loss_type; o.loss_scale = opt->loss_scale;
    o.grad_tol = opt->gradient_tol; o.step_tol = opt->step_tol; o.lambda0 = opt->initial_lambda;
    o.lambda_min = opt->min_lambda; o.lambda_max = opt->max_lambda;
    return o;
}

extern "C" {

void mdrp_destroy(mdrp_handle *h) {
    if (!h) return;
    DeviceGuard guard_(h->device);
    for (hipStream_t st : {h->stream, (hipStream_t)h->aux_stream, (hipStream_t)h->aux_stream2, (hipStream_t)h->copy_stream}) (void)hipStreamSynchronize(st);
    delete h;
}

int mdrp_synchronize(mdrp_handle *h) {
    if (!h) return MDRP_ERR_INVALID;
    MDRP_ENTER(h);
    HIPCHK(hipStreamSynchronize(h->stream));
    return MDRP_OK;
}

static int drain_and_return(mdrp_handle *h, int rc) {
    for (hipStream_t st : {h->stream, (hipStream_t)h->aux_stream, (hipStream_t)h->aux_stream2, (hipStream_t)h->copy_stream}) (void)hipStreamSynchronize(st);
    return rc;
}

static int estimate_async_locked(mdrp_handle *h, int kind, const double *x1, const double *x2, const double *d1, const double *d2, int batch, int n_max,
                                 const int32_t *n_per_pair, const mdrp_camera *cam1, const mdrp_camera *cam2, const mdrp_ransac_opt *ropt,
                                 const mdrp_bundle_opt *bopt, const uint64_t *budgets, int n_budgets, uint8_t *inlier_mask_dev) {
    const int rc = estimate_device(h, kind, x1, x2, d1, d2, batch, n_max, n_per_pair, cam1, cam2, ropt, bopt, inlier_mask_dev, nullptr, budgets, n_budgets);
    return rc ? drain_and_return(h, rc) : rc;
}
// ... 563 lines not shown
    if (batch > 0 && (!n_host || (ip->m_max > 0 && (!x1 || !x2 || !d1 || !d2 || !slot)))) { g_err = "mdrp_gather_image_pairs_ranked: NULL output"; return MDRP_ERR_INVALID; }
    MDRP_ENTER(h);
    int rc;
    if ((rc = h->fe_n.ensure(sizeof(int32_t) * std::max(batch, 1))) || (scores_dev && (rc = ensure_key_scratch(h, batch, ip->m_max)))) return rc;
    if ((rc = gather_images_device(h, ip, batch, x1, x2, d1, d2, slot, h->fe_n.as<int32_t>(), scores_dev, score_type))) return drain_and_return(h, rc);
    if ((rc = fetch_counts(h, batch))) return drain_and_return(h, rc);
    if (batch > 0) std::memcpy(n_host, h->fe_n_host, sizeof(int32_t) * batch);
    return MDRP_OK;
}

int mdrp_estimate_image_pairs_ranked_async(mdrp_handle *h, int kind, const mdrp_image_pairs *ip, const void *scores_dev, int score_type, int batch,
                                           const mdrp_camera *cam1, const mdrp_camera *cam2, const mdrp_ransac_opt *ropt, const mdrp_bundle_opt *bopt,
                                           uint8_t *match_mask_dev, int32_t *n_used_host) {
    if (!h || !ropt || !bopt) { g_err = "invalid argument"; return MDRP_ERR_INVALID; }
    if (int rc = check_front_end_kind(kind, "mdrp_estimate_image_pairs_ranked_async")) return rc;
    if (int rc = check_image_pairs(ip, batch)) return rc;
    if (int rc = check_score_type(scores_dev, score_type)) return rc;
    if (int rc = check_ranked_front_end(h, kind, batch, ip->m_max, cam1, cam2, ropt, bopt)) return rc;
    MDRP_ENTER(h);
    int rc;
    if ((rc = ensure_gather_buffers(h, batch, ip->m_max)) || (scores_dev && (rc = ensure_key_scratch(h, batch, ip->m_max)))) return rc;
    if ((rc = gather_images_device(h, ip, batch, h->fe_x1.as<double>(), h->fe_x2.as<double>(), h->fe_d1.as<double>(), h->fe_d2.as<double>(),
                                   h->fe_slot.as<int32_t>(), h->fe_n.as<int32_t>(), scores_dev, score_type)))
        return drain_and_return(h, rc);
    rc = estimate_gathered_ranked(h, kind, batch, ip->m_max, cam1, cam2, ropt, bopt, match_mask_dev, n_used_host);
    return rc ? drain_and_return(h, rc) : rc;
}

}

extern "C" {

int mdrp_last_sweep_stats(mdrp_handle *h, double *sweep_ms, int64_t *launches, int64_t *evaluations) {
    if (!h) return MDRP_ERR_INVALID;
    std::lock_guard<std::mutex> lock_(h->mu);
    if (sweep_ms) *sweep_ms = h->sweep_ms;
    if (launches) *launches = h->sweep_launches;
    if (evaluations) *evaluations = h->sweep_evals;
    return MDRP_OK;
}

int mdrp_last_stats_sized(mdrp_handle *h, mdrp_stats *out, size_t out_size) {
    if (!h || !out || out_size < sizeof(double)) return MDRP_ERR_INVALID;
    std::lock_guard<std::mutex> lock_(h->mu);
    mdrp_stats full, *caller = out;
    out = &full;
    out->count_ms = h->count_ms; out->count_launches = h->count_launches;
    out->sweep_ms = h->sweep_ms; out->sweep_launches = h->sweep_launches;
    out->evals_algorithmic = h->sweep_evals; out->evals_mfma = h->mfma_evals; out->evals_fp64 = h->fp64_evals; out->evals_bound = h->bound_evals;
    out->lo_ms = h->kind_ms[2]; out->lo_launches = h->kind_launches[2]; out->final_ms = h->kind_ms[3]; out->final_launches = h->kind_launches[3];
    out->bound_ms = h->kind_ms[4]; out->bound_launches = h->kind_launches[4]; out->solve_ms = h->kind_ms[5]; out->solve_launches = h->kind_launches[5];
    out->lm_cost_evals = h->lm_cost_evals; out->lm_accum_evals = h->lm_accum_evals;
    out->final_cost_evals = h->fin_cost_evals; out->final_accum_evals = h->fin_accum_evals;
    out->fuse_gate_timeouts = h->fuse_gate_timeouts; out->fuse_wait_timeouts = h->fuse_wait_timeouts;
    out->first_chunk = h->first_chunk;
    std::memcpy(caller, &full, std::min(out_size, sizeof full));
    return MDRP_OK;
}

int mdrp_last_stats(mdrp_handle *h, mdrp_stats *out) { return mdrp_last_stats_sized(h, out, offsetof(mdrp_stats, fuse_gate_timeouts)); }

int mdrp_solver_batch(mdrp_handle *h, int solver, const double *x1h, const double *x2h, const double *d1, const double *d2,
                      int count, mdrp_model *out, int32_t *n_out) {
    if (!h || count < 0 || solver < 0 || solver > 3 || !out || !n_out) { g_err = "invalid argument"; return MDRP_ERR_INVALID; }
    if (count == 0) return MDRP_OK;
    MDRP_ENTER(h);
    int rc;
    if ((rc = h->unit_a.ensure(sizeof(double) * 9 * count)) || (rc = h->unit_b.ensure(sizeof(double) * 9 * count)) ||
        (rc = h->unit_c.ensure(sizeof(double) * 3 * count)) || (rc = h->unit_d.ensure(sizeof(double) * 3 * count)) ||
        (rc = h->unit_e.ensure(sizeof(Model) * 4 * count)) || (rc = h->unit_f.ensure(sizeof(int32_t) * count)))
        return rc;
    hipStream_t s = h->stream;
    HIPCHK(hipMemcpyAsync(h->unit_a.p, x1h, sizeof(double) * 9 * count, hipMemcpyHostToDevice, s));
    HIPCHK(hipMemcpyAsync(h->unit_b.p, x2h, sizeof(double) * 9 * count, hipMemcpyHostToDevice, s));
    HIPCHK(hipMemcpyAsync(h->unit_c.p, d1, sizeof(double) * 3 * count, hipMemcpyHostToDevice, s));
    HIPCHK(hipMemcpyAsync(h->unit_d.p, d2, sizeof(double) * 3 * count, hipMemcpyHostToDevice, s));
    HIPCHK(hipMemsetAsync(h->unit_e.p, 0, sizeof(Model) * 4 * count, s));
    hipLaunchKernelGGL(k_solver_unit, dim3((count + 63) / 64), dim3(64), 0, s, solver, count, h->unit_a.as<double>(),
                       h->unit_b.as<double>(), h->unit_c.as<double>(), h->unit_d.as<double>(), h->unit_e.as<Model>(), h->unit_f.as<int32_t>());
    HIPCHK(hipGetLastError());
    HIPCHK(hipMemcpyAsync(out, h->unit_e.p, sizeof(Model) * 4 * count, hipMemcpyDeviceToHost, s));
    HIPCHK(hipMemcpyAsync(n_out, h->unit_f.p, sizeof(int32_t) * count, hipMemcpyDeviceToHost, s));
    HIPCHK(hipStreamSynchronize(s));
    return MDRP_OK;
}

int mdrp_classic_solver_batch(mdrp_handle *h, int kind, const double *x1h, const double *x2h, int count, mdrp_model *out, int32_t *n_out) {
    if (!h || count < 0 || kind < MDRP_RELPOSE_5PT || kind > MDRP_FUNDAMENTAL_7PT || !out || !n_out) { g_err = "invalid argument"; return MDRP_ERR_INVALID; }
    if (count == 0) return MDRP_OK;
    MDRP_ENTER(h);
    const int K = kind == MDRP_RELPOSE_5PT ? 5 : (kind == MDRP_SHARED_6PT ? 6 : 7), M = kind == MDRP_RELPOSE_5PT ? MAX_MODELS_5PT : (kind == MDRP_SHARED_6PT ? MAX_MODELS_6PT : 3);
    int rc;
    if ((rc = h->unit_a.ensure(sizeof(double) * 3 * K * count)) || (rc = h->unit_b.ensure(sizeof(double) * 3 * K * count)) ||
        (rc = h->unit_e.ensure(sizeof(Model) * M * count)) || (rc = h->unit_f.ensure(sizeof(int32_t) * count)))
        return rc;
    hipStream_t s = h->stream;
    HIPCHK(hipMemcpyAsync(h->unit_a.p, x1h, sizeof(double) * 3 * K * count, hipMemcpyHostToDevice, s));
    HIPCHK(hipMemcpyAsync(h->unit_b.p, x2h, sizeof(double) * 3 * K * count, hipMemcpyHostToDevice, s));
    HIPCHK(hipMemsetAsync(h->unit_e.p, 0, sizeof(Model) * M * count, s));
    if (kind == MDRP_SHARED_6PT)
        hipLaunchKernelGGL(kc_solver_unit<CLASSIC_SHARED>, dim3((count + 63) / 64), dim3(64), 0, s, count, h->unit_a.as<double>(),
                           h->unit_b.as<double>(), h->unit_e.as<Model>(), h->unit_f.as<int32_t>());
    else if (kind == MDRP_RELPOSE_5PT)
        hipLaunchKernelGGL(kc_solver_unit<CLASSIC_RELPOSE>, dim3((count + 63) / 64), dim3(64), SOLVE5_LDS_BYTES, s, count, h->unit_a.as<double>(),
                           h->unit_b.as<double>(), h->unit_e.as<Model>(), h->unit_f.as<int32_t>());
    else
        hipLaunchKernelGGL(kc_solver_unit<CLASSIC_FUND>, dim3((count + 63) / 64), dim3(64), SOLVE7_LDS_BYTES, s, count, h->unit_a.as<double>(),
                           h->unit_b.as<double>(), h->unit_e.as<Model>(), h->unit_f.as<int32_t>());
    HIPCHK(hipGetLastError());
    HIPCHK(hipMemcpyAsync(out, h->unit_e.p, sizeof(Model) * M * count, hipMemcpyDeviceToHost, s));
    HIPCHK(hipMemcpyAsync(n_out, h->unit_f.p, sizeof(int32_t) * count, hipMemcpyDeviceToHost, s));
    HIPCHK(hipStreamSynchronize(s));
    return MDRP_OK;
}

int mdrp_score_models(mdrp_handle *h, int kind, int mem_space, const mdrp_model *models, int num_models, const double *x1,
                      const double *x2, int n, double sq_threshold, double *scores, int32_t *counts) {
    if (!h || num_models < 0 || n < 0 || kind < 0 || kind > 5 || !scores || !counts) { g_err = "invalid argument"; return MDRP_ERR_INVALID; }
    if (num_models == 0) return MDRP_OK;
    MDRP_ENTER(h);
    hipStream_t s = h->stream;
    const int chunk = (num_models + 3) / 4;
    const size_t slots = (size_t)chunk * 4;
    int rc;
    if ((rc = h->pts.ensure(sizeof(double) * PT_STRIDE * std::max(n, 1))) || (rc = h->st.ensure(sizeof(PairState))) ||
        (rc = h->models.ensure(sizeof(Model) * slots)) || (rc = h->slot_score.ensure(sizeof(double) * slots)) ||
        (rc = h->slot_inl.ensure(sizeof(int32_t) * slots)) || (rc = h->tags[0].ensure(sizeof(uint32_t) * slots)) ||
        (rc = h->model_count[0].ensure(2 * sizeof(int32_t))))
        return rc;
    const double *x1d = x1, *x2d = x2;
    const Model *md = reinterpret_cast<const Model *>(models);
    if (mem_space == MDRP_MEM_HOST) {
        if ((rc = h->in_x1.ensure(sizeof(double) * 2 * std::max(n, 1))) || (rc = h->in_x2.ensure(sizeof(double) * 2 * std::max(n, 1)))) return rc;
        HIPCHK(hipMemcpyAsync(h->in_x1.p, x1, sizeof(double) * 2 * n, hipMemcpyHostToDevice, s));
        HIPCHK(hipMemcpyAsync(h->in_x2.p, x2, sizeof(double) * 2 * n, hipMemcpyHostToDevice, s));
        HIPCHK(hipMemcpyAsync(h->models.p, models, sizeof(Model) * num_models, hipMemcpyHostToDevice, s));
        x1d = h->in_x1.as<double>(); x2d = h->in_x2.as<double>();
        md = h->models.as<Model>();
    } else {
        HIPCHK(hipMemcpyAsync(h->models.p, models, sizeof(Model) * num_models, hipMemcpyDeviceToDevice, s));
        md = h->models.as<Model>();
    }
    if ((rc = upload_iota(s, h->tags[0].p, num_models))) return rc;
    const int32_t counts2[2] = {num_models, 0};
    HIPCHK(hipMemcpyAsync(h->model_count[0].p, counts2, 2 * sizeof(int32_t), hipMemcpyHostToDevice, s));
    if ((rc = stage_unit_pair(h, x1d, x2d, n, sq_threshold))) return rc;
    RunParams rp;
    std::memset(&rp, 0, sizeof rp);
    rp.kind = kind; rp.batch = 1; rp.n_max = std::max(n, 1); rp.chunk_len = chunk; rp.chunk_off = 0; rp.slot_stride = chunk * 4; rp.super_len = chunk;
    rp.mps = 4; rp.sample_sz = 3;
    const size_t tile_bytes = SCORE_TILE_BYTES;
    if ((rc = h->plan.ensure(sizeof(int32_t) * 8))) return rc;
    int32_t *plan = h->plan.as<int32_t>(), *totals = plan + 4;
    hipLaunchKernelGGL(k_plan, dim3(1), dim3(PLAN_THREADS), 0, s, 1, h->model_count[0].as<int32_t>(), plan, totals, SCORE_THREADS);
    const dim3 grid((unsigned)std::min(h->num_cu * 4, (num_models + SCORE_THREADS - 1) / SCORE_THREADS));
    h->ev_used = 0; h->sweep_launches = 1; h->sweep_evals = (int64_t)num_models * n;
    hipEvent_t e0, e1;
    if ((rc = get_events(h, &e0, &e1))) return rc;
    HIPCHK(hipEventRecord(e0, s));
    MDRP_SWEEP_DISPATCH(k_score, kind, grid, dim3(SCORE_THREADS), tile_bytes, s, rp, h->st.as<PairState>(), h->pts.as<double>(), md,
                        h->tags[0].as<uint32_t>(), h->model_count[0].as<int32_t>(), h->slot_score.as<double>(), h->slot_inl.as<int32_t>(), plan, totals);
    HIPCHK(hipEventRecord(e1, s));
    HIPCHK(hipGetLastError());
    const hipMemcpyKind back = mem_space == MDRP_MEM_HOST ? hipMemcpyDeviceToHost : hipMemcpyDeviceToDevice;
    HIPCHK(hipMemcpyAsync(scores, h->slot_score.p, sizeof(double) * num_models, back, s));
    HIPCHK(hipMemcpyAsync(counts, h->slot_inl.p, sizeof(int32_t) * num_models, back, s));
// ... 551 lines not shown
```

### mdrp_amd/csrc/mdrp_kernels.h

```cpp
#pragma once
#include <hip/hip_runtime.h>
#include <float.h>
#include "mdrp_logtab.h"
#include "mdrp_math.h"

#ifdef MDRP_SECONDARY_TU
#define MDRP_GLOBAL static __global__
#else
#define MDRP_GLOBAL __global__
#endif

namespace mdrp {

constexpr int PT_STRIDE = 6;
#define MDRP_TILE_PTS 512
#define MDRP_SCORE_MINWAVES 4
constexpr int TILE_PTS = MDRP_TILE_PTS;
constexpr size_t SCORE_TILE_BYTES = (size_t)TILE_PTS * (PT_STRIDE * sizeof(double) + 4 * sizeof(float));
#define MDRP_P1F_UNROLL 8
constexpr int PRUNE_EVERY = 4;
#define MDRP_DENSE_KEY 40
#define MDRP_SOLVE_MINWAVES 2
#define MDRP_SCORE_THREADS 256
constexpr int SCORE_THREADS = MDRP_SCORE_THREADS;
constexpr int LM_THREADS = 256;
constexpr int MAX_NP = 9;
constexpr int MAX_ACC = MAX_NP * (MAX_NP + 1) / 2 + MAX_NP;

struct PairState {
    int32_t n;
    int32_t table;
    int32_t active;
    int32_t n_triggers;
    double eps;
    double sq_thr;
    double scale_reproj;
    double lo_loss_scale;
    double final_loss_scale;
    double norm;
    double box[4];
    double cen[4];
    uint64_t best_min_cnt;
    double best_min_score;
    uint64_t dyn_max_iter;
    uint64_t iterations, refinements, num_inliers;
    double inlier_ratio, model_score;
    Model best;
};

struct Trigger {
    uint32_t iter;
    int32_t k_ref;
    int32_t k_min;
    int32_t cnt_min;
    double score_min;
    double ref_score;
    int32_t ref_cnt;
    int32_t cnt_ref;
    Model refined;
};

struct RunParams {
    int kind;
    int solver;
    int est_shift;
    int score_initial;
    int batch, n_max;
    int chunk_len;
    int chunk_off;
    int slot_stride;
    int mps;
    int sample_sz;
    int super_len;
    uint64_t chunk_start;
    uint64_t max_iterations, min_iterations;
    double dyn_mult, log_prob_missing;
    double weight_sampson;
    int final_max_it, final_loss;
    double grad_tol, step_tol, lambda0, lambda_min, lambda_max;
    int32_t *inl_stat;
    int ck_pairs, ck_plane;
};

constexpr int MAX_BUDGETS = 16;
struct FinalRows { int rec, out; };
__device__ __forceinline__ FinalRows final_rows(const RunParams &rp, int problem) {
    if (!rp.ck_pairs) return {problem, problem};
// ... 276 lines not shown
    if (n < 3) return;
    uint64_t state = table_state[t];
    __syncthreads();
    samples_block<3>(n, state, chunk_len, samples + (size_t)t * chunk_len * 3,
                     [](uint64_t n_, uint64_t &s_, uint32_t *o) { draw_sample3(n_, s_, o[0], o[1], o[2]); });
    if (threadIdx.x == 0) table_state[t] = state;
}

struct SampsonTerms { double C2, den; };

__device__ __forceinline__ double fma3(double a, double b, double c) {
#if defined(__HIP_DEVICE_COMPILE__)
    double d;
    asm("v_fma_f64 %0, %1, %2, %3" : "=v"(d) : "v"(a), "v"(b), "v"(c));
    return d;
#else
    return fma(a, b, c);
#endif
}

__device__ __forceinline__ SampsonTerms sampson_terms(const double E[9], double a, double b, double c, double d) {
    const double e0 = fma(E[0], a, fma3(E[1], b, E[2]));
    const double e1 = fma(E[3], a, fma3(E[4], b, E[5]));
    const double e2 = fma(E[6], a, fma3(E[7], b, E[8]));
    const double g0 = fma(E[0], c, fma3(E[3], d, E[6]));
    const double g1 = fma(E[1], c, fma3(E[4], d, E[7]));
    const double C = fma(c, e0, fma(d, e1, e2));
    SampsonTerms r;
    r.den = fma(e0, e0, fma(e1, e1, fma(g0, g0, g1 * g1)));
    r.C2 = C * C;
    return r;
}

__device__ __forceinline__ void bound_setup(const double E[9], const PairState &ps, double thr, float Ef[9], float &tb) {
    double thr_dmax;
    filter_setup(E, ps.box, thr, Ef, tb, thr_dmax);
}

template <bool POSE, bool RAWF>
__device__ __forceinline__ void model_matrix(const Model &m, double E[9], double R[9]) {
    if (RAWF) {
#pragma unroll
        for (int q = 0; q < 9; ++q) E[q] = reinterpret_cast<const double *>(&m)[q];
    } else {
        double Em[9];
        quat_to_R(m.q, R);
        essential_from_Rt(R, m.t, Em);
        if (POSE) {
#pragma unroll
            for (int q = 0; q < 9; ++q) E[q] = Em[q];
        } else fundamental_from_E(Em, m.f1, m.f2, E);
    }
}
template <bool POSE, bool RAWF>
__device__ __forceinline__ void model_matrix(const Model &m, double E[9]) {
    double R[9];
    model_matrix<POSE, RAWF>(m, E, R);
}

template <bool POSE>
__device__ __forceinline__ void model_pose(const Model *__restrict__ mp, double R[9], double t[3]) {
    if (POSE) {
        double q[4];
        q[0] = mp->q[0]; q[1] = mp->q[1]; q[2] = mp->q[2]; q[3] = mp->q[3];
        t[0] = mp->t[0]; t[1] = mp->t[1]; t[2] = mp->t[2];
        quat_to_R(q, R);
    }
}

__device__ __forceinline__ void store_rec32(float4 *__restrict__ recs32, int i, double a, double b, double c, double d) {
    float *q = reinterpret_cast<float *>(recs32) + (i >> 1) * 8 + (i & 1);
    q[0] = (float)a; q[2] = (float)b; q[4] = (float)c; q[6] = (float)d;
}

constexpr int PROBE_PTS = 64;

constexpr int solve_threads(int solver) { return solver == SOLVER_P3P || solver == SOLVER_SHIFT ? 256 : 64; }
template <int SOLVER>
__global__ __launch_bounds__(solve_threads(SOLVER), MDRP_SOLVE_MINWAVES) void k_solve(RunParams rp, const PairState *__restrict__ st, const uint32_t *__restrict__ samples,
                                               const double *__restrict__ pts, const double *__restrict__ dep,
                                               Model *__restrict__ models, int32_t *__restrict__ slot_inl,
                                               uint32_t *__restrict__ tags, int32_t *__restrict__ model_count,
                                               int it_begin, int it_end ) {
    const int pair = blockIdx.y;
    const int it = it_begin + blockIdx.x * solve_threads(SOLVER) + threadIdx.x;
    const PairState &ps = st[pair];
    if (!ps.active) return;
    const bool live = it < it_end;
    int n = 0;
    bool nan_model = false;
    Model out[4];
    auto load_sample = [&](Sample3 &s) {
        const uint32_t *sm = samples + ((size_t)ps.table * rp.chunk_len + it) * 3;
#pragma unroll
        for (int k = 0; k < 3; ++k) {
            const size_t idx = (size_t)pair * rp.n_max + sm[k];
            const double *p = pts + idx * PT_STRIDE;
            s.x1[k][0] = p[0]; s.x1[k][1] = p[1]; s.x2[k][0] = p[2]; s.x2[k][1] = p[3];
            s.d1[k] = dep[2 * idx]; s.d2[k] = dep[2 * idx + 1];
        }
    };
    if (live) {
        Sample3 s;
        load_sample(s);
        n = run_solver(SOLVER, s, out);
    }
    if (SOLVER == SOLVER_P3P) {
        const unsigned long long valid = __ballot(live && n > 0);
        const int first_valid = valid ? __ffsll((long long)valid) - 1 : 64;
        if (live && (int)(threadIdx.x & 63) < first_valid) {
            Sample3 s;
            load_sample(s);
            nan_model = p3p_reference_nan(s);
        }
    }
    const int lane = threadIdx.x & 63;
    int pre = n;
#pragma unroll
    for (int o = 1; o < 64; o <<= 1) {
        const int v = __shfl_up(pre, o, 64);
        if (lane >= o) pre += v;
    }
    const int tot = __shfl(pre, 63, 64);
    int base = 0;
    if (lane == 63 && tot > 0) base = atomicAdd(&model_count[2 * pair], tot);
    base = __shfl(base, 63, 64);
    if (!live) return;
    const size_t slot0 = (size_t)pair * rp.slot_stride + (size_t)(rp.chunk_off + it) * 4;
    int pos = base + pre - n;
    const size_t tag_base = (size_t)pair * rp.slot_stride;
    *reinterpret_cast<int4 *>(slot_inl + slot0) = make_int4(nan_model ? -3 : (n > 0 ? -2 : -1), n > 1 ? -2 : -1, n > 2 ? -2 : -1, n > 3 ? -2 : -1);
    if (nan_model) {
        Model m;
        model_identity(m);
        const double qnan = __longlong_as_double(0x7ff8000000000000ll);
        m.q[0] = m.q[1] = m.q[2] = m.q[3] = m.t[0] = m.t[1] = m.t[2] = m.scale = qnan;
        models[slot0] = m;
    }
#pragma unroll
    for (int k = 0; k < 4; ++k) {
        if (k < n) {
            models[slot0 + k] = out[k];
            tags[tag_base + pos] = (uint32_t)((rp.chunk_off + it) * 4 + k);
            ++pos;
        }
    }
}

template <bool POSE>
__device__ __forceinline__ bool record_inlier(const double *__restrict__ rec, const double E[9], const double R[9], const double t[3],
                                              double thr, double &r2) {
    const double2 *P = reinterpret_cast<const double2 *>(rec);
    const double2 p01 = P[0], p23 = P[1];
    const double a = p01.x, b = p01.y, c = p23.x, d = p23.y;
    const SampsonTerms s = sampson_terms(E, a, b, c, d);
    if (!(s.C2 < thr * (1.0 + 1e-12) * s.den)) return false;
    r2 = s.C2 / s.den;
    if (!(r2 < thr)) return false;
    if (POSE) {
        const double2 p45 = P[2];
        const double u0 = fma(R[0], a, fma(R[1], b, R[2]));
        const double u1 = fma(R[3], a, fma(R[4], b, R[5]));
        const double u2 = fma(R[6], a, fma(R[7], b, R[8]));
        const double uh = fma(u0, c, fma(u1, d, u2));
        const double ut = fma(u0, t[0], fma(u1, t[1], u2 * t[2]));
        const double ht = fma(c, t[0], fma(d, t[1], t[2]));
        const double A = -uh * p45.x * p45.y;
        const double b1 = -ut * p45.x, b2 = ht * p45.y;
        const double l1 = fma(-A, b2, b1), l2 = fma(-A, b1, b2);
        const double md = 0.01 * fma(-A, A, 1.0);
        return (l1 > md) && (l2 > md);
    }
    return true;
}

template <bool POSE>
__device__ __forceinline__ void score_point(const double *__restrict__ rec, const double E[9], const double R[9], const double t[3],
                                            double thr, double &score, int &cnt) {
    double r2;
    if (record_inlier<POSE>(rec, E, R, t, thr, r2)) { score += r2; ++cnt; }
}

struct Bar {
    long long rec_cnt;
    double rec_score;
    __device__ __forceinline__ explicit Bar(const PairState &ps)
        : rec_cnt((long long)ps.best_min_cnt), rec_score(ps.best_min_score < DBL_MAX ? ps.best_min_score * (1.0 + 1e-12) : DBL_MAX) {}
    __device__ __forceinline__ bool armed() const { return rec_score < DBL_MAX; }
    __device__ __forceinline__ bool out(int n, double thr, int processed, double score, int cnt) const {
        return ((long long)cnt + (long long)(n - processed) <= rec_cnt) && (score + thr * (double)(processed - cnt) >= rec_score);
    }
};
struct Prune : Bar {
    int n;
    int processed;
    bool dead;
    bool wave_dead;
    __device__ __forceinline__ Prune(const PairState &ps, bool live) : Bar(ps), n(ps.n), processed(0), dead(!live), wave_dead(false) {}
    __device__ __forceinline__ bool advance(int g, double thr, double score, int cnt) {
        processed += g;
        if (armed()) {
            dead = dead || out(n, thr, processed, score, cnt);
            if (__all(dead)) { wave_dead = true; return true; }
        }
        return false;
    }
};

__device__ __forceinline__ void write_slot(double *__restrict__ slot_score, int32_t *__restrict__ slot_inl, size_t at, bool pruned,
                                           double score, int cnt, int n, double thr) {
    slot_score[at] = pruned ? DBL_MAX : score + thr * (double)(n - cnt);
    slot_inl[at] = pruned ? -2 : cnt;
}

template <bool POSE>
__device__ __forceinline__ void score_tile_dense(const double *__restrict__ recs, int npts, const double E[9], const Model *__restrict__ mp,
                                                 double thr, double &score, int &cnt, Prune &pr) {
    double R[9], t[3] = {0, 0, 0};
#pragma unroll
    for (int i = 0; i < 9; ++i) R[i] = 0;
    model_pose<POSE>(mp, R, t);
    for (int p0 = 0; p0 < npts; p0 += 32 * PRUNE_EVERY) {
        const int g = min(32 * PRUNE_EVERY, npts - p0);
        if (!pr.dead) {
#pragma unroll 2
            for (int j = 0; j < g; ++j) score_point<POSE>(recs + (size_t)(p0 + j) * PT_STRIDE, E, R, t, thr, score, cnt);
        }
        if (pr.advance(g, thr, score, cnt)) return;
    }
}

typedef float f32x2 __attribute__((ext_vector_type(2)));
__device__ __forceinline__ f32x2 numerator2(const f32x2 Ev[9], const float4 ab, const float4 cd, f32x2 &e0, f32x2 &e1) {
    const f32x2 a = {ab.x, ab.y}, b = {ab.z, ab.w}, c = {cd.x, cd.y}, d = {cd.z, cd.w};
    e0 = __builtin_elementwise_fma(Ev[0], a, __builtin_elementwise_fma(Ev[1], b, Ev[2]));
    e1 = __builtin_elementwise_fma(Ev[3], a, __builtin_elementwise_fma(Ev[4], b, Ev[5]));
    const f32x2 e2 = __builtin_elementwise_fma(Ev[6], a, __builtin_elementwise_fma(Ev[7], b, Ev[8]));
    return __builtin_elementwise_fma(c, e0, __builtin_elementwise_fma(d, e1, e2));
}

template <bool POSE>
__device__ __forceinline__ void score_tile_f32(const double *__restrict__ recs, const float4 *__restrict__ recs32, int npts,
                                               const double E[9], const float Ef[9], float tb, const Model *__restrict__ mp,
                                               double thr, double &score, int &cnt, Prune &pr) {
    constexpr int WIN = 64;
    static_assert(TILE_PTS % WIN == 0, "window must divide the tile");
    f32x2 Ev[9];
#pragma unroll
    for (int i = 0; i < 9; ++i) Ev[i] = (f32x2)(Ef[i]);
    for (int p0 = 0; p0 < npts; p0 += WIN) {
        const int g = min(WIN, npts - p0);
        const double *base = recs + (size_t)p0 * PT_STRIDE;
        uint32_t half[2] = {0, 0};
#pragma unroll
        for (int h = 0; h < 2; ++h) {
            const int q0 = 32 * h;
            if (q0 < g) {
                const float4 *b32 = recs32 + p0 + q0;
                uint32_t mask = 0;
#pragma unroll 1
                for (int j0 = 0; j0 < 32; j0 += MDRP_P1F_UNROLL) {
#pragma unroll
                    for (int jj = 0; jj < MDRP_P1F_UNROLL; jj += 2) {
                        const int j = j0 + jj;
                        f32x2 e0, e1;
                        const f32x2 C = numerator2(Ev, b32[j], b32[j + 1], e0, e1);
                        const float cx = C.x, cy = C.y;
                        unsigned long long kx, ky, co;
                        asm("v_cmp_ngt_f32_e64 %0, |%1|, %2" : "=s"(kx) : "v"(cx), "v"(tb));
                        asm("v_cmp_ngt_f32_e64 %0, |%1|, %2" : "=s"(ky) : "v"(cy), "v"(tb));
                        asm("v_addc_co_u32_e64 %0, %1, %0, %0, %2" : "+v"(mask), "=s"(co) : "s"(kx));
                        asm("v_addc_co_u32_e64 %0, %1, %0, %0, %2" : "+v"(mask), "=s"(co) : "s"(ky));
                    }
                }
// ... 209 lines not shown
                     "v_add_f32 %0, %0, %2\n\t"
                     "v_add_f32 %1, %1, %6\n\t"
                     "v_add_f32 %0, %0, %4\n\t"
                     "v_add_f32 %1, %1, %8"
                     : "+v"(cand[t0]), "+v"(cand[t0 + 1]), "=&v"(d0), "=&v"(d1), "=&v"(d2), "=&v"(d3), "=&v"(d4), "=&v"(d5), "=&v"(d6), "=&v"(d7)
                     : "v"(acc[t0][0]), "v"(acc[t0][1]), "v"(acc[t0][2]), "v"(acc[t0][3]), "v"(acc[t0 + 1][0]), "v"(acc[t0 + 1][1]),
                       "v"(acc[t0 + 1][2]), "v"(acc[t0 + 1][3]), "v"(tbv[t0]), "v"(tbv[t0 + 1]));
    };
    const int G = (n + 15) >> 4;
    const uint4 *A = rfrag + (size_t)pair * ((rp.n_max + 15) >> 4) * 64;
    const int n_tiles = (G + A_TILE_GROUPS - 1) / A_TILE_GROUPS;
    const int t_split = phase == 0 ? n_tiles : count_split_tiles(ps, n_tiles, cand_stat, pair);
    const int t_lo = phase == 2 ? t_split : 0, t_hi = phase == 1 ? t_split : n_tiles;
    uint4 stage[4];
    auto fetch = [&](int tile) {
        const int g0 = tile * A_TILE_GROUPS;
#pragma unroll
        for (int k = 0; k < 4; ++k) {
            const int idx = k * CNT_THREADS + tid;
            stage[k] = (g0 + (idx >> 6)) < G ? A[(size_t)g0 * 64 + idx] : make_uint4(0u, 0u, 0u, 0u);
        }
    };
    auto commit = [&](int buf) {
#pragma unroll
        for (int k = 0; k < 4; ++k) s_lds[buf * A_TILE_GROUPS * 64 + k * CNT_THREADS + tid] = stage[k];
    };
    if (t_lo >= t_hi) return;
    fetch(t_lo);
    commit(t_lo & 1);
    __syncthreads();
    for (int tile = t_lo; tile < t_hi; ++tile) {
        const int buf = tile & 1;
        if (tile + 1 < t_hi) fetch(tile + 1);
        if (!idle) {
            const uint4 *T = s_lds + buf * A_TILE_GROUPS * 64 + lane;
            uint4 f0 = T[0], f1 = T[64];
#pragma unroll
            for (int t = 0; t < CNT_TILES; t += 2) mfma2(f0, t);
#pragma unroll
            for (int g = 0; g < A_TILE_GROUPS; g += 2) {
                f0 = T[(size_t)min(g + 2, A_TILE_GROUPS - 1) * 64];
#pragma unroll
                for (int t = 0; t < CNT_TILES; t += 2) { test2(t); mfma2(f1, t); }
                f1 = T[(size_t)min(g + 3, A_TILE_GROUPS - 1) * 64];
                if (g + 2 < A_TILE_GROUPS) {
#pragma unroll
                    for (int t = 0; t < CNT_TILES; t += 2) { test2(t); mfma2(f0, t); }
                } else {
#pragma unroll
                    for (int t = 0; t < CNT_TILES; t += 2) test2(t);
                }
            }
        }
        if (tile + 1 < t_hi) commit(buf ^ 1);
        __syncthreads();
    }
    if (idle) return;
    uint32_t *s_out = reinterpret_cast<uint32_t *>(&s_frag[wave][0][0]);
    const int swept = (t_hi - t_lo) * A_TILE_GROUPS * 16, real = min(max(n - t_lo * A_TILE_GROUPS * 16, 0), swept);
    const int pad = swept - real;
    const bool split_a = phase == 1 && t_hi < n_tiles;
    const int rest = split_a ? n - t_hi * A_TILE_GROUPS * 16 : 0;
#pragma unroll
    for (int t = 0; t < CNT_TILES; ++t) {
        float o = cand[t];
        o += __shfl_xor(o, 16, 64);
        o += __shfl_xor(o, 32, 64);
        if (ksl == 0) s_out[16 * t + col] = (uint32_t)((int)o - pad);
    }
    __builtin_amdgcn_fence(__ATOMIC_RELEASE, "wavefront");
    __builtin_amdgcn_wave_barrier();
    const Bar bar(ps);
#pragma unroll
    for (int r = 0; r < CNT_ROUNDS; ++r) {
        const int i = m0 + 64 * r + lane;
        const bool live = i < cnt;
        const int cnd_here = live ? (int)s_out[64 * r + lane] + part_r[r] : 0;
        const int cnd = cnd_here + rest;
        if (cand_stat && phase == 1 && !split_a && bar.rec_cnt == 0 && !(ps.best_min_score < DBL_MAX)) {
            const int tot = wave_sum_i(cnd_here), lv = __popcll(__ballot(live));
            if (lane == 0 && lv) { atomicAdd(&cand_stat[2 * pair], (unsigned long long)tot); atomicAdd(&cand_stat[2 * pair + 1], (unsigned long long)lv * (unsigned long long)n); }
        }
        if (cand_out && live) cand_out[i] = cnd;
        const bool surv = live && ((long long)cnd > bar.rec_cnt || thr * (double)(n - cnd) < bar.rec_score);
        const unsigned long long ball = __ballot(surv);
        if (ball) {
            int base = 0;
            const int first = __ffsll((long long)ball) - 1;
            if (lane == first) base = atomicAdd(split_a ? &und_count[2 * pair] : &surv_count[pair], __popcll(ball));
            base = __shfl(base, first, 64);
            if (surv) {
                const size_t at = slot_base + base + __popcll(ball & ((1ull << lane) - 1ull));
                if (split_a) { tags_und[at] = slot_r[r]; und_part[at] = cnd_here; }
                else {
                    const uint32_t key = (uint32_t)min(PROBE_PTS, (int)(((long long)cnd * PROBE_PTS + n - 1) / n));
                    tags_surv[at] = slot_r[r] | (key << 24);
                }
            }
        }
    }
    if (stats && lane == 0 && wave == 0 && blk == 0) {
        if (phase != 2) atomicAdd(&stats[0], (unsigned long long)cnt * (unsigned long long)n);
        atomicAdd(&stats[1], (unsigned long long)(((cnt + 15) / 16) * 16) * (unsigned long long)swept);
    }
}

constexpr int BND_THREADS = 256;
#define MDRP_BND_TILE 256
constexpr int BND_TILE = MDRP_BND_TILE;

template <bool POSE, bool RAWF = false>
__global__ __launch_bounds__(BND_THREADS, 4) void k_bound(RunParams rp, const PairState *__restrict__ st, const double *__restrict__ pts,
                                                          const Model *__restrict__ models, const uint32_t *__restrict__ tags_in,
                                                          const int32_t *__restrict__ cnt_in, const int32_t *__restrict__ plan,
                                                          uint32_t *__restrict__ tags_out,
                                                          int32_t *__restrict__ cnt_out, unsigned long long *__restrict__ stats,
                                                          double *__restrict__ dbg_lb = nullptr ,
                                                          int32_t *__restrict__ dbg_cnt_ub = nullptr) {
    __shared__ float4 s_rec[BND_TILE];
    struct Open { uint32_t tag; int32_t sane; float Ef[9], eC, eD, thr_dn, c0, c1; double lb; };
    __shared__ Open s_open[BND_THREADS];
    __shared__ int s_wave_open[BND_THREADS / 64];
    const int total = plan[rp.batch];
    const int w = blockIdx.x;
    if (w >= total) return;
    const int pair = plan_find(plan, rp.batch, w);
    const int blk = w - plan[pair];
    const PairState &ps = st[pair];
    const int n = ps.n, cnt = cnt_in[pair];
    const int tid = threadIdx.x, lane = tid & 63, wave = tid >> 6;
    const int i = blk * BND_THREADS + tid;
    bool open = i < cnt;
    const size_t slot_base = (size_t)pair * rp.slot_stride;
    const double thr = ps.sq_thr;
    uint32_t tag = 0;
    float Ef[9], eC = 0.f, eD = 1.f, thr_dn = 0.f;
    bool sane = false;
#pragma unroll
    for (int q = 0; q < 9; ++q) Ef[q] = 0.f;
    if (open) {
        tag = tags_in[slot_base + i];
        const Model m = models[slot_base + (tag & 0xFFFFFFu)];
        double E[9];
        model_matrix<POSE, RAWF>(m, E);
        sane = bound_setup32(E, ps.box, thr, Ef, eC, eD, thr_dn);
    }
    double total_lb = 0.0;
    f32x2 cnt2 = {0.f, 0.f};
    const float thr_cnt = (float)(thr * (1.0 + 1e-5)) * (1.0f + 1e-6f);
    const float BIG = 1.2089258e24f;
    const f32x2 nbig = {-BIG, -BIG}, kcnt = {thr_cnt * BIG, thr_cnt * BIG};
    const Bar bar(ps);
    float4 *s_pair = s_rec;
    const double *gp = pts + (size_t)pair * rp.n_max * PT_STRIDE;
    for (int t0 = 0; t0 < n; t0 += BND_TILE) {
        const int npts = min(BND_TILE, n - t0);
        __syncthreads();
        for (int j = tid; j < npts; j += BND_THREADS) {
            const double2 *src = reinterpret_cast<const double2 *>(gp + (size_t)(t0 + j) * PT_STRIDE);
            const double2 p0 = src[0], p1 = src[1];
            store_rec32(s_pair, j, p0.x, p0.y, p1.x, p1.y);
        }
        __syncthreads();
        if (__ballot(open)) {
            f32x2 Ev[9];
#pragma unroll
            for (int q = 0; q < 9; ++q) Ev[q] = (f32x2){Ef[q], Ef[q]};
// ... 65 lines not shown
        dbg_cnt_ub[tag & 0xFFFFFFu] = sane ? (int32_t)min((long long)n, (long long)(cnt2.x + cnt2.y) + 1) : n;
    }
    const unsigned long long ball = __ballot(surv);
    if (ball) {
        int base = 0;
        const int first = __ffsll((long long)ball) - 1;
        if (lane == first) base = atomicAdd(&cnt_out[pair], __popcll(ball));
        base = __shfl(base, first, 64);
        if (surv) tags_out[slot_base + base + __popcll(ball & ((1ull << lane) - 1ull))] = tag;
    }
    if (stats && tid == 0 && blk == 0) atomicAdd(stats, (unsigned long long)cnt * (unsigned long long)n);
}

MDRP_GLOBAL __launch_bounds__(256) void k_sort_tags(RunParams rp, const PairState *__restrict__ st, int32_t *__restrict__ model_count,
                                                   const int32_t *__restrict__ surv_count,
                                                   const uint32_t *__restrict__ tags, uint32_t *__restrict__ tags_sorted) {
    const int pair = blockIdx.x, tid = threadIdx.x;
    const PairState &ps = st[pair];
    if (!ps.active) return;
    __shared__ int s_hist[PROBE_PTS + 1], s_pos[PROBE_PTS + 1];
    __shared__ int s_dense;
    if (tid <= PROBE_PTS) s_hist[tid] = 0;
    if (tid == 0) s_dense = 0;
    __syncthreads();
    const int cnt = surv_count[pair];
    const size_t slot_base = (size_t)pair * rp.slot_stride;
    const uint32_t *src = tags + slot_base;
    uint32_t *dst = tags_sorted + slot_base;
    const int dense_min = ps.n >= 8 ? MDRP_DENSE_KEY : PROBE_PTS + 1;
    for (int i = tid; i < cnt; i += 256) atomicAdd(&s_hist[min(src[i] >> 24, (uint32_t)PROBE_PTS)], 1);
    __syncthreads();
    if (tid < 64) {
        const int v = tid < dense_min ? s_hist[tid] : 0;
        int incl = v;
#pragma unroll
        for (int o = 1; o < 64; o <<= 1) {
            const int u = __shfl_up(incl, o, 64);
            if (tid >= o) incl += u;
        }
        s_pos[tid] = incl - v;
        if (tid == 63) s_pos[64] = incl;
    }
    __syncthreads();
    const int cap = rp.slot_stride;
    for (int i = tid; i < cnt; i += 256) {
        const uint32_t t = src[i];
        const int key = (int)min(t >> 24, (uint32_t)PROBE_PTS);
        if (key >= dense_min) dst[cap - 1 - atomicAdd(&s_dense, 1)] = t & 0xFFFFFFu;
        else dst[atomicAdd(&s_pos[key], 1)] = t & 0xFFFFFFu;
    }
    __syncthreads();
    if (tid == 0) { model_count[2 * pair] = cnt - s_dense; model_count[2 * pair + 1] = s_dense; }
}

MDRP_GLOBAL __launch_bounds__(PLAN_THREADS) void k_plan(int batch, const int32_t *__restrict__ model_count, int32_t *__restrict__ plan,
                                                       int32_t *__restrict__ totals , int per_wg) {
    __shared__ int s_w[PLAN_THREADS / 64 + 1];
    int run_d = 0, run_s = 0;
    int32_t *pd = plan, *psp = plan + batch + 1;
    for (int p0 = 0; p0 < batch; p0 += PLAN_THREADS) {
        const int p = p0 + threadIdx.x;
        int bd = 0, bs = 0;
        if (p < batch) {
            bs = (model_count[2 * p] + per_wg - 1) / per_wg;
            bd = (model_count[2 * p + 1] + per_wg - 1) / per_wg;
        }
        int tot_d, tot_s;
        const int ed = plan_block_scan(bd, tot_d, s_w), es = plan_block_scan(bs, tot_s, s_w);
        if (p < batch) { pd[p] = run_d + run_s + ed + es; psp[p] = bs; }
        run_d += tot_d;
        run_s += tot_s;
    }
    if (threadIdx.x == 0) { pd[batch] = run_d + run_s; psp[batch] = 0; totals[0] = run_d; totals[1] = run_d + run_s; totals[2] = 0; }
}

template <bool POSE, bool RAWF = false>
__global__ __launch_bounds__(SCORE_THREADS, MDRP_SCORE_MINWAVES) void k_score(RunParams rp, const PairState *__restrict__ st, const double *__restrict__ pts,
                                                         const Model *__restrict__ models, const uint32_t *__restrict__ tags,
                                                         const int32_t *__restrict__ model_count, double *__restrict__ slot_score,
                                                         int32_t *__restrict__ slot_inl, const int32_t *__restrict__ plan,
                                                         int32_t *__restrict__ totals) {
    extern __shared__ double tile[];
    float4 *tile32 = reinterpret_cast<float4 *>(tile + TILE_PTS * PT_STRIDE);
    const int total = totals[1];
    const int tid = threadIdx.x;
    for (int w = blockIdx.x; w < total; w += gridDim.x) {
    const SweepItem item = sweep_item(rp, plan, model_count, tags, w, SCORE_THREADS, tid);
    const int pair = item.pair;
    const bool dense = item.dense, live = item.live;
    const PairState &ps = st[pair];
    const int n = ps.n;
    const double thr = ps.sq_thr;
    double E[9];
    float tb, Ef[9];
    const Model *mp = models + item.slot_base + item.slot;
#pragma unroll
    for (int i = 0; i < 9; ++i) E[i] = 0;
    if (live) model_matrix<POSE, RAWF>(*mp, E);
    bound_setup(E, ps, thr, Ef, tb);
    double score = 0;
    int cnt = 0;
    Prune pr(ps, live);
    const double *gp = pts + (size_t)pair * rp.n_max * PT_STRIDE;
    for (int t0 = 0; t0 < n; t0 += TILE_PTS) {
        const int npts = min(TILE_PTS, n - t0);
        __syncthreads();
        {
            const double2 *src = reinterpret_cast<const double2 *>(gp + (size_t)t0 * PT_STRIDE);
            double2 *dst = reinterpret_cast<double2 *>(tile);
            for (int i = tid; i < npts; i += SCORE_THREADS) {
                const double2 p0 = src[3 * i], p1 = src[3 * i + 1], p2 = src[3 * i + 2];
                dst[3 * i] = p0; dst[3 * i + 1] = p1; dst[3 * i + 2] = p2;
                if (!dense) store_rec32(tile32, i, p0.x, p0.y, p1.x, p1.y);
            }
        }
        __syncthreads();
        if (!pr.wave_dead) {
            if (dense) score_tile_dense<POSE>(tile, npts, E, mp, thr, score, cnt, pr);
            else score_tile_f32<POSE>(tile, tile32, npts, E, Ef, tb, mp, thr, score, cnt, pr);
        }
    }
    if (live) write_slot(slot_score, slot_inl, item.slot_base + item.slot, pr.dead, score, cnt, n, thr);
    }
}

constexpr int SCORE_WAVE_MAX_PAIRS = 128;
constexpr int SCW_THREADS = 256;
template <bool POSE, bool RAWF = false>
__global__ __launch_bounds__(SCW_THREADS) void k_score_w(RunParams rp, const PairState *__restrict__ st, const double *__restrict__ pts,
                                                         const Model *__restrict__ models, const uint32_t *__restrict__ tags ,
                                                         const int32_t *__restrict__ model_count, double *__restrict__ slot_score,
                                                         int32_t *__restrict__ slot_inl, const int32_t *__restrict__ plan ) {
    __shared__ double s_r2[SCW_THREADS / 64][64];
    const int total = plan[rp.batch];
    const int lane = threadIdx.x & 63, wave = threadIdx.x >> 6;
    const unsigned long long lt = (1ull << lane) - 1ull;
    for (int w = blockIdx.x; w < total; w += gridDim.x) {
        const int pair = plan_find(plan, rp.batch, w);
        const int i = (w - plan[pair]) * (SCW_THREADS / 64) + wave;
        const int cnt_sparse = model_count[2 * pair], cnt_dense = model_count[2 * pair + 1];
        if (i >= cnt_sparse + cnt_dense) continue;
        const PairState &ps = st[pair];
        const int n = ps.n;
        const double thr = ps.sq_thr;
        const size_t slot_base = (size_t)pair * rp.slot_stride;
        const uint32_t slot = tags[slot_base + (i < cnt_sparse ? i : rp.slot_stride - 1 - (i - cnt_sparse))];
        const Model m = models[slot_base + slot];
        double E[9], R[9], t[3] = {m.t[0], m.t[1], m.t[2]};
#pragma unroll
        for (int q = 0; q < 9; ++q) R[q] = 0;
        model_matrix<POSE, RAWF>(m, E, R);
        const Bar bar(ps);
        const double *gp = pts + (size_t)pair * rp.n_max * PT_STRIDE;
        double score = 0;
        int cnt = 0;
        bool pruned = false;
        for (int t0 = 0; t0 < n; t0 += 64) {
            const int r = t0 + lane;
            double s1 = 0;
            int c1 = 0;
            if (r < n) score_point<POSE>(gp + (size_t)r * PT_STRIDE, E, R, t, thr, s1, c1);
            const unsigned long long ball = __ballot(c1 != 0);
            if (ball) {
                if (c1) s_r2[wave][__popcll(ball & lt)] = s1;
                __builtin_amdgcn_fence(__ATOMIC_RELEASE, "wavefront");
                __builtin_amdgcn_wave_barrier();
                __builtin_amdgcn_fence(__ATOMIC_ACQUIRE, "wavefront");
                const int k = __popcll(ball);
                for (int j = 0; j < k; ++j) score += s_r2[wave][j];
                cnt += k;
                __builtin_amdgcn_wave_barrier();
            }
            const int processed = min(t0 + 64, n);
            if (bar.armed() && ((processed & 127) == 0 || processed == n) && bar.out(n, thr, processed, score, cnt)) { pruned = true; break; }
        }
        if (lane == 0) write_slot(slot_score, slot_inl, slot_base + slot, pruned, score, cnt, n, thr);
    }
}

constexpr int SPLIT_THREADS = 256;
constexpr int SPLIT_WAVES = SPLIT_THREADS / 64;
constexpr int SPLIT_HYP = 64;
constexpr int SPLIT_Q = 8;
constexpr int SPLIT_STEP = SPLIT_WAVES * SPLIT_Q;
static_assert(128 % SPLIT_STEP == 0, "the bail-out positions (every 128 records) must be step boundaries");
template <bool POSE, bool RAWF = false>
__global__ __launch_bounds__(SPLIT_THREADS, MDRP_SCORE_MINWAVES) void k_score_split(RunParams rp, const PairState *__restrict__ st, const double *__restrict__ pts,
                                                               const Model *__restrict__ models, const uint32_t *__restrict__ tags ,
                                                               const int32_t *__restrict__ model_count, double *__restrict__ slot_score,
                                                               int32_t *__restrict__ slot_inl, const int32_t *__restrict__ plan ,
                                                               const int32_t *__restrict__ totals) {
    __shared__ double s_rec[2][SPLIT_WAVES][SPLIT_Q * PT_STRIDE];
    __shared__ float4 s_rec32[2][SPLIT_WAVES][SPLIT_Q];
    __shared__ double s_r2[2][SPLIT_STEP][SPLIT_HYP];
    __shared__ int32_t s_cnt[2][SPLIT_WAVES][SPLIT_HYP];
    __shared__ unsigned long long s_dead[2];
    const int total = totals[1];
    const int lane = threadIdx.x & 63;
    const int wave = __builtin_amdgcn_readfirstlane(threadIdx.x >> 6);
    for (int w = blockIdx.x; w < total; w += gridDim.x) {
        const SweepItem item = sweep_item(rp, plan, model_count, tags, w, SPLIT_HYP, lane);
        const int pair = item.pair;
        const bool dense = item.dense, live = item.live;
        const PairState &ps = st[pair];
        const int n = ps.n;
        const double thr = ps.sq_thr;
        double E[9], R[9], t[3] = {0, 0, 0};
#pragma unroll
        for (int q = 0; q < 9; ++q) { E[q] = 0; R[q] = 0; }
        if (live) {
            const Model m = models[item.slot_base + item.slot];
            model_matrix<POSE, RAWF>(m, E, R);
            if (!RAWF) { t[0] = m.t[0]; t[1] = m.t[1]; t[2] = m.t[2]; }
        }
        float Ef[9], tb;
        bound_setup(E, ps, thr, Ef, tb);
        const Bar bar(ps);
        const double *gp = pts + (size_t)pair * rp.n_max * PT_STRIDE;
        const int steps = (n + SPLIT_STEP - 1) / SPLIT_STEP;
        double2 nx = {0, 0};
        auto fetch = [&](int j) {
            const int r = j * SPLIT_STEP + wave * SPLIT_Q + lane / 3;
            if (lane < 3 * SPLIT_Q && r < n) nx = reinterpret_cast<const double2 *>(gp + (size_t)r * PT_STRIDE)[lane % 3];
        };
        auto stage = [&](int j) {
            const int k = lane / 3, part = lane % 3;
            if (lane < 3 * SPLIT_Q && j * SPLIT_STEP + wave * SPLIT_Q + k < n) {
                reinterpret_cast<double2 *>(s_rec[j & 1][wave])[lane] = nx;
                float *q = reinterpret_cast<float *>(s_rec32[j & 1][wave]) + (k >> 1) * 8 + (k & 1);
                if (part == 0) { q[0] = (float)nx.x; q[2] = (float)nx.y; }
                else if (part == 1) { q[4] = (float)nx.x; q[6] = (float)nx.y; }
            }
        };
        fetch(0);
        stage(0);
        __syncthreads();
        double score = 0;
        int cnt = 0;
        bool dead = !live;
        bool skip = !live;
        for (int j = 0; j <= steps; ++j) {
            if (j > 0) {
                const unsigned long long dm = s_dead[(j - 1) & 1];
                if (dm == ~0ull) break;
                skip = (dm >> lane) & 1;
            }
            if (wave == 0) {
                if (j > 0) {
                    const int b = (j - 1) & 1;
                    if (!dead) {
#pragma unroll 1
                        for (int q = 0; q < SPLIT_WAVES; ++q) {
#pragma unroll
                            for (int r = 0; r < SPLIT_Q; ++r) score += s_r2[b][q * SPLIT_Q + r][lane];
                            cnt += s_cnt[b][q][lane];
                        }
                    }
                    const int processed = min(j * SPLIT_STEP, n);
                    if (bar.armed() && ((processed & 127) == 0 || processed == n)) dead = dead || bar.out(n, thr, processed, score, cnt);
                }
                if (j < steps) {
                    const unsigned long long dm = __ballot(dead);
                    if (lane == 0) s_dead[j & 1] = dm;
                }
                skip = dead;
            }
            if (j == steps) break;
            if (j + 1 < steps) fetch(j + 1);
            const int b = j & 1;
            const int valid = min(SPLIT_Q, n - (j * SPLIT_STEP + wave * SPLIT_Q));
            const double *rec = s_rec[b][wave];
            double *out = &s_r2[b][wave * SPLIT_Q][lane];
            int found = 0;
            if (dense) {
#pragma unroll 2
                for (int jj = 0; jj < SPLIT_Q; ++jj) {
                    double v = 0.0, r2;
                    if (jj < valid && !skip && record_inlier<POSE>(rec + jj * PT_STRIDE, E, R, t, thr, r2)) { v = r2; ++found; }
                    out[jj * SPLIT_HYP] = v;
                }
            } else {
#pragma unroll
                for (int jj = 0; jj < SPLIT_Q; ++jj) out[jj * SPLIT_HYP] = 0.0;
                const float4 *b32 = s_rec32[b][wave];
                f32x2 Ev[9];
#pragma unroll
                for (int q = 0; q < 9; ++q) Ev[q] = (f32x2)(Ef[q]);
                uint32_t mask = 0;
#pragma unroll
                for (int jj = 0; jj < SPLIT_Q; jj += 2) {
                    f32x2 e0, e1;
                    const f32x2 C = numerator2(Ev, b32[jj], b32[jj + 1], e0, e1);
                    mask |= (!(fabsf(C.x) > tb) ? 1u : 0u) << jj;
                    mask |= (!(fabsf(C.y) > tb) ? 1u : 0u) << (jj + 1);
                }
                mask &= valid >= SPLIT_Q ? 0xFFu : (valid > 0 ? (1u << valid) - 1u : 0u);
                if (skip) mask = 0;
                while (mask) {
                    const int jj = __ffs(mask) - 1;
                    mask &= mask - 1;
                    double r2;
                    if (record_inlier<POSE>(rec + jj * PT_STRIDE, E, R, t, thr, r2)) { out[jj * SPLIT_HYP] = r2; ++found; }
                }
            }
            s_cnt[b][wave][lane] = found;
            if (j + 1 < steps) stage(j + 1);
            __syncthreads();
        }
        if (wave == 0 && live) write_slot(slot_score, slot_inl, item.slot_base + item.slot, dead, score, cnt, n, thr);
    }
}

template <int MPS = 4, int IPL = 1>
__global__ __launch_bounds__(64) void k_scan(RunParams rp, PairState *__restrict__ st, const double *__restrict__ slot_score,
                                             const int32_t *__restrict__ slot_inl, Trigger *__restrict__ triggers,
                                             int trig_cap, const int32_t *__restrict__ model_count,
                                             unsigned long long *__restrict__ evals) {
    const int pair = blockIdx.x, lane = threadIdx.x;
    PairState &ps = st[pair];
    if (!ps.active) { if (lane == 0) ps.n_triggers = 0; return; }
    if (lane == 0 && evals) atomicAdd(evals, (unsigned long long)(model_count[2 * pair] + model_count[2 * pair + 1]) * (unsigned long long)ps.n);
    long long run_cnt = (long long)ps.best_min_cnt;
    double run_score = ps.best_min_score;
    const double nan_score = (double)ps.n * ps.sq_thr;
    int ntrig = rp.chunk_off > 0 ? ps.n_triggers : 0;
    static_assert(MPS % 4 == 0, "slots of an iteration are read as 16-byte groups");
    constexpr int NG = MPS / 4;
    const size_t slot_base = (size_t)pair * rp.slot_stride + (size_t)rp.chunk_off * MPS;
    struct Slots { int4 c[IPL][NG]; double2 s01[IPL][NG], s23[IPL][NG]; };
    auto fetch = [&](int it0) {
        Slots r;
#pragma unroll
        for (int j = 0; j < IPL; ++j) {
            const int it = it0 + IPL * lane + j;
#pragma unroll
            for (int g = 0; g < NG; ++g) {
                if (it < rp.chunk_len) {
                    r.c[j][g] = *reinterpret_cast<const int4 *>(slot_inl + slot_base + (size_t)it * MPS + 4 * g);
                    const double2 *sp = reinterpret_cast<const double2 *>(slot_score + slot_base + (size_t)it * MPS + 4 * g);
                    r.s01[j][g] = sp[0]; r.s23[j][g] = sp[1];
                } else { r.c[j][g] = make_int4(-1, -1, -1, -1); r.s01[j][g] = r.s23[j][g] = make_double2(DBL_MAX, DBL_MAX); }
            }
        }
        return r;
    };
    Slots nxt = fetch(0);
    for (int it0 = 0; it0 < rp.chunk_len; it0 += 64 * IPL) {
        const Slots cur = nxt;
        if (it0 + 64 * IPL < rp.chunk_len) nxt = fetch(it0 + 64 * IPL);
        int c[IPL][MPS];
        double s[IPL][MPS];
        long long lc = -1;
        double ls = DBL_MAX;
#pragma unroll
        for (int j = 0; j < IPL; ++j) {
#pragma unroll
            for (int g = 0; g < NG; ++g) {
                c[j][4 * g] = cur.c[j][g].x; c[j][4 * g + 1] = cur.c[j][g].y; c[j][4 * g + 2] = cur.c[j][g].z; c[j][4 * g + 3] = cur.c[j][g].w;
                s[j][4 * g] = c[j][4 * g] >= 0 ? cur.s01[j][g].x : DBL_MAX; s[j][4 * g + 1] = c[j][4 * g + 1] >= 0 ? cur.s01[j][g].y : DBL_MAX;
                s[j][4 * g + 2] = c[j][4 * g + 2] >= 0 ? cur.s23[j][g].x : DBL_MAX; s[j][4 * g + 3] = c[j][4 * g + 3] >= 0 ? cur.s23[j][g].y : DBL_MAX;
            }
            if (c[j][0] == -3) { c[j][0] = 0; s[j][0] = nan_score; }
#pragma unroll
            for (int k = 0; k < MPS; ++k) if (c[j][k] >= 0) { lc = max(lc, (long long)c[j][k]); ls = fmin(ls, s[j][k]); }
        }
        if (__all(lc <= run_cnt && !(ls < run_score))) continue;
        long long pc = lc;
        double psn = ls;
#pragma unroll
        for (int o = 1; o < 64; o <<= 1) {
            const long long vc = __shfl_up(pc, o, 64);
            const double vs = __shfl_up(psn, o, 64);
            if (lane >= o) { pc = max(pc, vc); psn = fmin(psn, vs); }
        }
        const long long tot_c = __shfl(pc, 63, 64);
        const double tot_s = __shfl(psn, 63, 64);
        long long ec = __shfl_up(pc, 1, 64);
        double es = __shfl_up(psn, 1, 64);
        if (lane == 0) { ec = -1; es = DBL_MAX; }
        long long bc = max(run_cnt, ec);
        double bs = fmin(run_score, es);
        int k_ref[IPL], k_min[IPL], cnt_min[IPL], cnt_ref[IPL], mine = 0;
        double score_min[IPL];
#pragma unroll
        for (int j = 0; j < IPL; ++j) {
            k_ref[j] = -1; k_min[j] = -1; cnt_min[j] = 0; cnt_ref[j] = 0; score_min[j] = 0;
#pragma unroll
            for (int k = 0; k < MPS; ++k) {
                if (c[j][k] >= 0) {
                    const bool more = (long long)c[j][k] > bc, better = s[j][k] < bs;
                    if (more || better) {
                        if (more) bc = c[j][k];
                        if (better) { bs = s[j][k]; k_min[j] = k; score_min[j] = s[j][k]; cnt_min[j] = c[j][k]; }
// ... 900 lines not shown
```

### mdrp_amd/csrc/mdrp_schedule.h

```cpp
#pragma once
#include "../../include/mdrp.h"

#include <algorithm>
#include <cmath>
#include <cstdint>
#include <cstdlib>
#include <map>
#include <string>
#include <vector>

namespace mdrp {
namespace sched {

constexpr int NC_MAX = 8;

inline int model_slots(int kind) { return kind == MDRP_RELPOSE_5PT ? 12 : (kind == MDRP_SHARED_6PT ? 16 : 4); }
inline int sample_size(int kind) { return kind == MDRP_RELPOSE_5PT ? 5 : (kind == MDRP_SHARED_6PT ? 6 : (kind == MDRP_FUNDAMENTAL_7PT ? 7 : 3)); }

inline uint64_t certain_iterations(uint64_t max_iterations, uint64_t min_iterations) {
    return max_iterations == 0 ? 1 : std::min<uint64_t>(max_iterations, min_iterations + 1);
}
inline int chunk_capacity(uint64_t max_iterations, uint64_t min_iterations) {
    const uint64_t cap = std::min<uint64_t>(std::max<uint64_t>(max_iterations, 1), std::max<uint64_t>(min_iterations + 1, 4096));
    return (int)std::min<uint64_t>(cap, 16384);
// ... 1 lines not shown

struct Lead {
    int n = 0;
    uint64_t len[NC_MAX - 1] = {};
    uint64_t first() const { return n ? len[0] : 0; }
};

inline bool parse_chunks(const char *spec_or_null, Lead &lead) {
    lead = Lead{};
    if (!spec_or_null) return false;
    const std::string spec = spec_or_null;
    size_t pos = 0;
    while (pos < spec.size() && lead.n < NC_MAX - 1) {
        const size_t q = spec.find(',', pos);
        const long v = atol(spec.substr(pos, q == std::string::npos ? std::string::npos : q - pos).c_str());
        if (v > 0) lead.len[lead.n++] = (uint64_t)v;
        if (q == std::string::npos) break;
        pos = q + 1;
    }
    return true;
}

constexpr uint64_t LEAD_5PT_MAX = 512;
constexpr uint64_t LEAD_BUDGET = LEAD_5PT_MAX;
inline Lead default_lead(int kind, uint64_t certain, double seen_wish) {
    const uint64_t sixteenth = std::max<uint64_t>(128, certain / 16 / 64 * 64);
    Lead lead;
    lead.n = 1;
    if (kind == MDRP_FUNDAMENTAL_7PT) { lead.n = 2; lead.len[0] = 128; lead.len[1] = 1024; }
    else if (kind == MDRP_SHARED_6PT) lead.len[0] = 128;
    else if (kind == MDRP_RELPOSE_5PT) lead.len[0] = std::min<uint64_t>(LEAD_5PT_MAX, sixteenth);
    else {
        lead.len[0] = std::min<uint64_t>(256, sixteenth);
        if (seen_wish >= 0.0 && certain >= 8192) lead.len[0] = (uint64_t)std::min(1024.0, std::max(128.0, std::ceil(seen_wish / 64.0) * 64.0));
    }
    return lead;
}

struct Layout {
    int n_chunks = 1;
    uint64_t lens[NC_MAX] = {};
    int offs[NC_MAX] = {};
    uint64_t super_len = 0;
};
inline Layout super_chunk_layout(uint64_t it0, uint64_t certain, int chunk_cap, const Lead &lead, uint64_t max_needed, uint64_t max_iterations) {
    Layout l;
    if (it0 < certain) {
        const uint64_t span = std::min<uint64_t>(certain - it0, (uint64_t)chunk_cap);
        uint64_t used = 0;
        l.n_chunks = 0;
        if (it0 == 0)
            for (int i = 0; i < lead.n; ++i) {
                if (used + 2 * lead.len[i] > span) break;
                l.lens[l.n_chunks++] = lead.len[i]; used += lead.len[i];
            }
        l.lens[l.n_chunks++] = span - used;
    } else {
        l.lens[0] = std::min<uint64_t>(std::min<uint64_t>(std::max<uint64_t>(max_needed, 256), max_iterations - it0), (uint64_t)chunk_cap);
    }
    for (int c = 0; c < l.n_chunks; ++c) l.super_len += l.lens[c];
    for (int c = 1; c < l.n_chunks; ++c) l.offs[c] = l.offs[c - 1] + (int)l.lens[c - 1];
    return l;
}

inline void group_tables(const int32_t *n_per_pair, int batch, std::vector<int32_t> &table_of, std::vector<int32_t> &tab_n) {
    table_of.assign(batch, 0); tab_n.clear();
    std::map<int32_t, int32_t> ids;
    for (int i = 0; i < batch; ++i) {
        auto it = ids.find(n_per_pair[i]);
        if (it == ids.end()) { it = ids.emplace(n_per_pair[i], (int32_t)tab_n.size()).first; tab_n.push_back(n_per_pair[i]); }
        table_of[i] = it->second;
    }
}

inline int pairs_per_pass(size_t free_bytes, size_t per_pair, int batch) {
    const size_t budget = std::min<size_t>((size_t)(0.5 * (double)free_bytes), (size_t)96 << 30);
    const int per_pass = (int)std::max<size_t>(1, std::min<size_t>((size_t)batch, budget / per_pair));
    return std::min(per_pass, 65535);
}

inline int lo_lanes(int batch_call, int n_max) { return (batch_call >= 128 && n_max < 4096) ? 64 : 256; }
inline int final_lanes(int batch_call) { return batch_call >= 4096 ? 64 : 256; }

inline long long fuse_n_scale(int n_max) { return std::max(1, (n_max + 1999) / 2000); }
inline int fuse_gate_us(int batch, int n_max) { return (int)std::min<long long>((50000 + 40ll * batch) * fuse_n_scale(n_max), 200000); }
inline int fuse_wait_us(int batch, int n_max) { return (int)std::min<long long>((20000 + 4ll * batch) * fuse_n_scale(n_max), 100000); }

}
}
```

Measured before the change: 129,700.

## Add first-pick prefix scoring filter and LDS-reserved solver residency

Result: faster. 134,100, median of 6 (+3.4%).

```diff
diff --git a/include/mdrp.h b/include/mdrp.h
--- a/include/mdrp.h
+++ b/include/mdrp.h
@@ -100,6 +100,9 @@
 
 int mdrp_solver_batch(mdrp_handle *h, int solver, const double *x1h, const double *x2h, const double *d1,
                       const double *d2, int count, mdrp_model *out, int32_t *n_out);
+
+int mdrp_solver_residency(int device, int solver, int resident_per_simd, uint64_t keep_free_bytes, uint64_t *lds_per_cu,
+                          uint64_t *reserve_bytes, int *workgroups_per_cu);
 
 int mdrp_classic_solver_batch(mdrp_handle *h, int kind, const double *x1h, const double *x2h, int count, mdrp_model *out,
                               int32_t *n_out);
diff --git a/mdrp_amd/_capi.py b/mdrp_amd/_capi.py
--- a/mdrp_amd/_capi.py
+++ b/mdrp_amd/_capi.py
@@ -15,7 +15,7 @@
 EXPORTS = (
     "mdrp_create_", "mdrp_create_on_stream_", "mdrp_destroy", "mdrp_last_error", "mdrp_version", "mdrp_abi_version", "mdrp_hip_build_version", "mdrp_synchronize", "mdrp_estimate_batch",
     "mdrp_estimate_batch_async", "mdrp_fetch_results", "mdrp_copy_results_device", "mdrp_solver_batch", "mdrp_score_models", "mdrp_count_candidates", "mdrp_bound_models", "mdrp_refine_models",
-    "mdrp_last_sweep_stats", "mdrp_last_stats", "mdrp_last_stats_sized", "mdrp_classic_solver_batch",
+    "mdrp_last_sweep_stats", "mdrp_last_stats", "mdrp_last_stats_sized", "mdrp_classic_solver_batch", "mdrp_solver_residency",
     "mdrp_gather_matches", "mdrp_estimate_matches_async",
     "mdrp_estimate_batch_budgets", "mdrp_estimate_batch_budgets_async", "mdrp_fetch_budget_results", "mdrp_copy_budget_results_device",
     "mdrp_refine_batch", "mdrp_refine_batch_async",
@@ -194,6 +194,8 @@
                                                vp, vp, vp, vp, vp]
         if hasattr(lib, "mdrp_replay_slots"):
             lib.mdrp_replay_slots.argtypes = [vp, C.POINTER(RansacOpt), C.POINTER(Replay)]
+        if hasattr(lib, "mdrp_solver_residency"):
+            lib.mdrp_solver_residency.argtypes = [C.c_int, C.c_int, C.c_int, C.c_uint64, C.POINTER(C.c_uint64), C.POINTER(C.c_uint64), C.POINTER(C.c_int)]
         _lib = lib
         return lib
 
@@ -258,6 +260,15 @@
         raise ValueError(f"ransac_opt['max_iterations'] = {ro['max_iterations']} differs from the last budget {ks[-1]}")
     ro["max_iterations"] = ks[-1]
     return np.asarray(ks, dtype=np.uint64), ro
+
+
+def solver_residency(solver, resident_per_simd, keep_free_bytes=0, device=0):
+    lib = load_library()
+    if not hasattr(lib, "mdrp_solver_residency"):
+        raise MdrpError("this library has no mdrp_solver_residency")
+    lds, reserve, wgs = C.c_uint64(), C.c_uint64(), C.c_int()
+    _check(lib, lib.mdrp_solver_residency(int(device), int(solver), int(resident_per_simd), int(keep_free_bytes), C.byref(lds), C.byref(reserve), C.byref(wgs)))
+    return lds.value, reserve.value, wgs.value
 
 
 def library_version():
diff --git a/mdrp_amd/build.py b/mdrp_amd/build.py
--- a/mdrp_amd/build.py
+++ b/mdrp_amd/build.py
@@ -12,7 +12,7 @@
         os.path.join(HERE, "csrc", "mdrp_classic.h"), os.path.join(HERE, "csrc", "mdrp_classic_math.h"),
         os.path.join(HERE, "csrc", "mdrp_logtab.h"), os.path.join(HERE, "csrc", "mdrp_instances.h"),
         os.path.join(HERE, "csrc", "mdrp_frontend.h"), os.path.join(HERE, "csrc", "mdrp_schedule.h"),
-        os.path.join(HERE, "csrc", "mdrp_from_model.h"), os.path.join(HERE, "csrc", "mdrp_prior.h"), os.path.join(HERE, "csrc", "mdrp_prosac.h"),
+        os.path.join(HERE, "csrc", "mdrp_front.h"), os.path.join(HERE, "csrc", "mdrp_from_model.h"), os.path.join(HERE, "csrc", "mdrp_prior.h"), os.path.join(HERE, "csrc", "mdrp_prosac.h"),
         os.path.join(HERE, "..", "include", "mdrp.h")]
 OUT = os.path.join(HERE, "libmdrp_hip.so")
 _MARK = b"MDRP_SRC_HASH="
diff --git a/mdrp_amd/csrc/mdrp_capi.hip b/mdrp_amd/csrc/mdrp_capi.hip
--- a/mdrp_amd/csrc/mdrp_capi.hip
+++ b/mdrp_amd/csrc/mdrp_capi.hip
@@ -135,6 +135,7 @@
     DevBuf fuse;
     Event ev_lo, ev_tables, ev_sampled[2], ev_solved[sched::NC_MAX], ev_scanned[sched::NC_MAX];
     int num_cu = 256;
+    size_t lds_per_cu = 65536;
     DevBuf pts, dep, st;
     DevBuf params;
     Pinned<unsigned char> params_host;
@@ -406,6 +407,8 @@
     const bool lo_overlap = env_int("MDRP_LO_OVERLAP", 1) != 0;
     const bool use_bound = env_int("MDRP_BOUND", 1) != 0;
     const bool score_split = env_int("MDRP_SCORE_SPLIT", 1) != 0;
+    const int first_pick = sched::first_pick(kind, batch_call, SCORE_WAVE_MAX_PAIRS, env_int("MDRP_FIRST_PICK", -1));
+    const int solve_resident = env_int("MDRP_SOLVE_RESIDENT", -1);
     const int lo_threads = env_int("MDRP_LO_THREADS", sched::lo_lanes(batch_call, n_max));
     const int final_threads = env_int("MDRP_FINAL_THREADS", sched::final_lanes(batch_call));
     const int samp_threads = env_int("MDRP_SAMPLE_THREADS", ssz == 3 ? SAMP_THREADS : (ssz == 5 ? 512 : 256));
@@ -573,6 +576,14 @@
         return v;
     }
 
+    size_t solve_reserve(const ChunkView &v) const {
+        const bool beside_front = piped && it0 == 0 && v.c == 1 && kind == MDRP_CALIB;
+        if (!beside_front || solve_resident == 0 || (solve_resident < 0 && first_pick == 0)) return 0;
+        const size_t sweep_wg = std::max<size_t>(SPLIT_LDS_BYTES, std::max<size_t>(SCORE_TILE_BYTES, CNT_LDS_BYTES));
+        return solve_resident > 0 ? sched::solver_reservation(h->lds_per_cu, solve_resident, 0)
+                                  : sched::solver_reservation(h->lds_per_cu, sched::SOLVE_RESIDENT, 2 * sweep_wg);
+    }
+
     int solve(const ChunkView &v, hipStream_t st_) {
         const RunParams &r = v.r;
         const int pc = v.pc;
@@ -599,8 +610,12 @@
                 hipLaunchKernelGGL(kc_solve<CLASSIC_FUND>, sgrid, dim3(64), SOLVE7_LDS_BYTES, st_, r, v.st, v.samples, v.pts, v.models, v.slot_inl, v.tags, v.model_count);
             return MDRP_OK;
         }
+        const size_t reserve = solve_reserve(v);
 #define MDRP_SOLVE_LAUNCH(S)                                                                                                   \
-    hipLaunchKernelGGL(k_solve<S>, dim3((r.chunk_len + solve_threads(S) - 1) / solve_threads(S), pc), dim3(solve_threads(S)), 0, st_, r, v.st, v.samples, v.pts, v.dep, v.models, v.slot_inl, v.tags, v.model_count, 0, r.chunk_len)
+    do {                                                                                                                       \
+        const int threads_ = reserve ? 64 : solve_threads(S);                                                                  \
+        hipLaunchKernelGGL(k_solve<S>, dim3((r.chunk_len + threads_ - 1) / threads_, pc), dim3(threads_), reserve, st_, r, v.st, v.samples, v.pts, v.dep, v.models, v.slot_inl, v.tags, v.model_count, 0, r.chunk_len); \
+    } while (0)
         switch (r.solver) {
         case SOLVER_P3P: MDRP_SOLVE_LAUNCH(SOLVER_P3P); break;
         case SOLVER_SHIFT: MDRP_SOLVE_LAUNCH(SOLVER_SHIFT); break;
@@ -653,6 +668,27 @@
         return MDRP_OK;
     }
 
+    int front(const ChunkView &v, Survivors &sv) {
+        if (!(v.first_of_run && first_pick > 0)) return MDRP_OK;
+        uint32_t *tags_pick = v.tags, *tags_rest = v.tags_sorted_other;
+        int32_t *plan = h->plan.as<int32_t>(), *totals = plan + 2 * (size_t)batch + 2;
+        hipLaunchKernelGGL(k_first_pick, dim3(v.pc), dim3(FIRST_THREADS), 0, s, v.r, v.st, sv.count, sv.tags, first_pick, tags_pick, v.surv2, tags_rest, v.und_count);
+        hipLaunchKernelGGL(k_sort_tags, dim3(v.pc), dim3(256), 0, s, v.r, v.st, v.model_count, v.surv2, tags_pick, v.tags_sorted);
+        hipLaunchKernelGGL(k_plan, dim3(1), dim3(PLAN_THREADS), 0, s, v.pc, v.model_count, plan, totals, SPLIT_HYP);
+        hipEvent_t f0, f1;
+        if (int rc = get_events(h, &f0, &f1, 0)) return rc;
+        HIPCHK(hipEventRecord(f0, s));
+        const long long ub = 2ll * v.pc;
+        MDRP_SWEEP_DISPATCH(k_first_score, kind, dim3((unsigned)std::min(ub, (long long)h->num_cu * 32)), dim3(SPLIT_THREADS), 0, s, v.r, v.st, v.pts, v.models,
+                            v.tags_sorted, v.model_count, v.slot_score, v.slot_inl, plan, totals);
+        HIPCHK(hipEventRecord(f1, s));
+        h->sweep_launches++;
+        hipLaunchKernelGGL(k_first_filter, dim3(v.pc), dim3(FIRST_THREADS), 0, s, v.r, v.st, v.slot_score, v.slot_inl, tags_pick, v.surv2, tags_rest, v.und_count,
+                           v.tags_v, v.surv1, &cnt->progress.evals_sweep);
+        sv = Survivors{v.tags_v, v.surv1};
+        return MDRP_OK;
+    }
+
     int score(const ChunkView &v, const Survivors &sv, hipEvent_t e0, hipEvent_t e1) {
         const bool wave = batch_call <= SCORE_WAVE_MAX_PAIRS, split = !wave && score_split && !v.first_of_run;
         const int models = v.r.chunk_len * mps;
@@ -688,7 +724,7 @@
         hipEvent_t e0, e1;
         Survivors sv;
         int rc;
-        if ((rc = get_events(h, &e0, &e1, 0)) || (rc = count(v)) || (rc = bound(v, sv)) || (rc = score(v, sv, e0, e1))) return rc;
+        if ((rc = get_events(h, &e0, &e1, 0)) || (rc = count(v)) || (rc = bound(v, sv)) || (rc = front(v, sv)) || (rc = score(v, sv, e0, e1))) return rc;
         scan(v);
         return MDRP_OK;
     }
@@ -1048,6 +1084,7 @@
     hipDeviceProp_t prop;
     HIPCHK(hipGetDeviceProperties(&prop, device));
     h->num_cu = prop.multiProcessorCount > 0 ? prop.multiProcessorCount : 256;
+    if (prop.maxSharedMemoryPerMultiProcessor > 0) h->lds_per_cu = prop.maxSharedMemoryPerMultiProcessor;
     HIPCHK(hipHostMalloc((void **)&h->progress_host.v, sizeof(Progress), hipHostMallocDefault));
     HIPCHK(hipHostMalloc((void **)&h->lm_stats_host.v, LM_STATS_BYTES, hipHostMallocDefault));
     HIPCHK(hipHostMalloc((void **)&h->wish_host.v, 2 * sizeof(int32_t), hipHostMallocDefault));
@@ -1777,6 +1814,23 @@
     HIPCHK(hipMemcpyAsync(out, h->unit_e.p, sizeof(Model) * 4 * count, hipMemcpyDeviceToHost, s));
     HIPCHK(hipMemcpyAsync(n_out, h->unit_f.p, sizeof(int32_t) * count, hipMemcpyDeviceToHost, s));
     HIPCHK(hipStreamSynchronize(s));
+    return MDRP_OK;
+}
+
+int mdrp_solver_residency(int device, int solver, int resident_per_simd, uint64_t keep_free_bytes, uint64_t *lds_per_cu, uint64_t *reserve_bytes,
+                          int *workgroups_per_cu) {
+    if (!lds_per_cu || !reserve_bytes || !workgroups_per_cu || solver < SOLVER_P3P || solver > SOLVER_VARYING) { g_err = "mdrp_solver_residency: bad argument"; return MDRP_ERR_INVALID; }
+    int ndev = 0;
+    if (hipGetDeviceCount(&ndev) != hipSuccess || ndev <= 0 || device < 0 || device >= ndev) { g_err = "no usable HIP device"; return MDRP_ERR_NO_DEVICE; }
+    DeviceGuard guard_(device);
+    if (!guard_.ok) { g_err = "hipSetDevice failed"; return MDRP_ERR_HIP; }
+    hipDeviceProp_t prop;
+    HIPCHK(hipGetDeviceProperties(&prop, device));
+    *lds_per_cu = (uint64_t)prop.maxSharedMemoryPerMultiProcessor;
+    *reserve_bytes = (uint64_t)sched::solver_reservation((size_t)*lds_per_cu, resident_per_simd, (size_t)keep_free_bytes);
+    const void *fn = solver == SOLVER_P3P ? reinterpret_cast<const void *>(k_solve<SOLVER_P3P>) : solver == SOLVER_SHIFT ? reinterpret_cast<const void *>(k_solve<SOLVER_SHIFT>)
+                   : solver == SOLVER_SHARED ? reinterpret_cast<const void *>(k_solve<SOLVER_SHARED>) : reinterpret_cast<const void *>(k_solve<SOLVER_VARYING>);
+    HIPCHK(hipOccupancyMaxActiveBlocksPerMultiprocessor(workgroups_per_cu, fn, 64, (size_t)*reserve_bytes));
     return MDRP_OK;
 }
 
diff --git a/mdrp_amd/csrc/mdrp_front.h b/mdrp_amd/csrc/mdrp_front.h
--- /dev/null
+++ b/mdrp_amd/csrc/mdrp_front.h
@@ -0,0 +1,33 @@
+#pragma once
+#include <cfloat>
+#include <cstdint>
+#include "mdrp_math.h"
+
+namespace mdrp {
+
+struct RecordBar {
+    long long rec_cnt;
+    double rec_score;
+    MDRP_HD RecordBar(long long cnt, double raw_score) : rec_cnt(cnt), rec_score(raw_score < DBL_MAX ? raw_score * (1.0 + 1e-12) : DBL_MAX) {}
+    MDRP_HD bool armed() const { return rec_score < DBL_MAX; }
+    MDRP_HD bool out(int n, double thr, int processed, double score, int cnt) const {
+        return ((long long)cnt + (long long)(n - processed) <= rec_cnt) && (score + thr * (double)(processed - cnt) >= rec_score);
+    }
+    MDRP_HD bool retires(int n, double thr, int cand) const { return !((long long)cand > rec_cnt || thr * (double)(n - cand) < rec_score); }
+};
+
+MDRP_HD RecordBar prefix_bar(const int32_t *iter_p, const int32_t *cnt_p, const double *score_p, int np, int iter) {
+    long long rc = -1;
+    double rs = DBL_MAX;
+    for (int j = 0; j < np; ++j) {
+        if (iter_p[j] < iter && cnt_p[j] >= 0) {
+            if ((long long)cnt_p[j] > rc) rc = cnt_p[j];
+            if (score_p[j] < rs) rs = score_p[j];
+        }
+    }
+    return RecordBar(rc, rs);
+}
+
+MDRP_HD int cand_of_key(int key, int n) { return (int)(((long long)key * n) >> 6); }
+
+}
diff --git a/mdrp_amd/csrc/mdrp_kernels.h b/mdrp_amd/csrc/mdrp_kernels.h
--- a/mdrp_amd/csrc/mdrp_kernels.h
+++ b/mdrp_amd/csrc/mdrp_kernels.h
@@ -3,6 +3,7 @@
 #include <float.h>
 #include "mdrp_logtab.h"
 #include "mdrp_math.h"
+#include "mdrp_front.h"
 
 #ifdef MDRP_SECONDARY_TU
 #define MDRP_GLOBAL static __global__
@@ -445,8 +446,9 @@
                                                Model *__restrict__ models, int32_t *__restrict__ slot_inl,
                                                uint32_t *__restrict__ tags, int32_t *__restrict__ model_count,
                                                int it_begin, int it_end ) {
+    extern __shared__ unsigned char solve_reserved[];
     const int pair = blockIdx.y;
-    const int it = it_begin + blockIdx.x * solve_threads(SOLVER) + threadIdx.x;
+    const int it = it_begin + blockIdx.x * blockDim.x + threadIdx.x;
     const PairState &ps = st[pair];
     if (!ps.active) return;
     const bool live = it < it_end;
@@ -544,15 +546,8 @@
     if (record_inlier<POSE>(rec, E, R, t, thr, r2)) { score += r2; ++cnt; }
 }
 
-struct Bar {
-    long long rec_cnt;
-    double rec_score;
-    __device__ __forceinline__ explicit Bar(const PairState &ps)
-        : rec_cnt((long long)ps.best_min_cnt), rec_score(ps.best_min_score < DBL_MAX ? ps.best_min_score * (1.0 + 1e-12) : DBL_MAX) {}
-    __device__ __forceinline__ bool armed() const { return rec_score < DBL_MAX; }
-    __device__ __forceinline__ bool out(int n, double thr, int processed, double score, int cnt) const {
-        return ((long long)cnt + (long long)(n - processed) <= rec_cnt) && (score + thr * (double)(processed - cnt) >= rec_score);
-    }
+struct Bar : RecordBar {
+    __device__ __forceinline__ explicit Bar(const PairState &ps) : RecordBar((long long)ps.best_min_cnt, ps.best_min_score) {}
 };
 struct Prune : Bar {
     int n;
@@ -928,7 +923,7 @@
             if (lane == 0 && lv) { atomicAdd(&cand_stat[2 * pair], (unsigned long long)tot); atomicAdd(&cand_stat[2 * pair + 1], (unsigned long long)lv * (unsigned long long)n); }
         }
         if (cand_out && live) cand_out[i] = cnd;
-        const bool surv = live && ((long long)cnd > bar.rec_cnt || thr * (double)(n - cnd) < bar.rec_score);
+        const bool surv = live && !bar.retires(n, thr, cnd);
         const unsigned long long ball = __ballot(surv);
         if (ball) {
             int base = 0;
@@ -1160,6 +1155,7 @@
                                                          int32_t *__restrict__ totals) {
     extern __shared__ double tile[];
     float4 *tile32 = reinterpret_cast<float4 *>(tile + TILE_PTS * PT_STRIDE);
+    __builtin_amdgcn_s_setprio(3);
     const int total = totals[1];
     const int tid = threadIdx.x;
     for (int w = blockIdx.x; w < total; w += gridDim.x) {
@@ -1200,6 +1196,7 @@
     }
     if (live) write_slot(slot_score, slot_inl, item.slot_base + item.slot, pr.dead, score, cnt, n, thr);
     }
+    __builtin_amdgcn_s_setprio(0);
 }
 
 constexpr int SCORE_WAVE_MAX_PAIRS = 128;
@@ -1261,13 +1258,16 @@
 constexpr int SPLIT_HYP = 64;
 constexpr int SPLIT_Q = 8;
 constexpr int SPLIT_STEP = SPLIT_WAVES * SPLIT_Q;
+constexpr size_t SPLIT_LDS_BYTES = 2 * SPLIT_WAVES * SPLIT_Q * (PT_STRIDE * sizeof(double) + sizeof(float4)) + 2 * SPLIT_STEP * SPLIT_HYP * sizeof(double) +
+                                   2 * SPLIT_WAVES * SPLIT_HYP * sizeof(int32_t) + 2 * sizeof(unsigned long long);
+constexpr size_t CNT_LDS_BYTES = 2 * 16 * 64 * sizeof(uint4);
 static_assert(128 % SPLIT_STEP == 0, "the bail-out positions (every 128 records) must be step boundaries");
-template <bool POSE, bool RAWF = false>
-__global__ __launch_bounds__(SPLIT_THREADS, MDRP_SCORE_MINWAVES) void k_score_split(RunParams rp, const PairState *__restrict__ st, const double *__restrict__ pts,
-                                                               const Model *__restrict__ models, const uint32_t *__restrict__ tags ,
-                                                               const int32_t *__restrict__ model_count, double *__restrict__ slot_score,
-                                                               int32_t *__restrict__ slot_inl, const int32_t *__restrict__ plan ,
-                                                               const int32_t *__restrict__ totals) {
+template <bool POSE, bool RAWF>
+__device__ __forceinline__ void score_split_items(const RunParams &rp, const PairState *__restrict__ st, const double *__restrict__ pts,
+                                                  const Model *__restrict__ models, const uint32_t *__restrict__ tags ,
+                                                  const int32_t *__restrict__ model_count, double *__restrict__ slot_score,
+                                                  int32_t *__restrict__ slot_inl, const int32_t *__restrict__ plan ,
+                                                  const int32_t *__restrict__ totals) {
     __shared__ double s_rec[2][SPLIT_WAVES][SPLIT_Q * PT_STRIDE];
     __shared__ float4 s_rec32[2][SPLIT_WAVES][SPLIT_Q];
     __shared__ double s_r2[2][SPLIT_STEP][SPLIT_HYP];
@@ -1387,6 +1387,121 @@
         }
         if (wave == 0 && live) write_slot(slot_score, slot_inl, item.slot_base + item.slot, dead, score, cnt, n, thr);
     }
+}
+template <bool POSE, bool RAWF = false>
+__global__ __launch_bounds__(SPLIT_THREADS, MDRP_SCORE_MINWAVES) void k_score_split(RunParams rp, const PairState *__restrict__ st, const double *__restrict__ pts,
+                                                               const Model *__restrict__ models, const uint32_t *__restrict__ tags,
+                                                               const int32_t *__restrict__ model_count, double *__restrict__ slot_score,
+                                                               int32_t *__restrict__ slot_inl, const int32_t *__restrict__ plan,
+                                                               const int32_t *__restrict__ totals) {
+    score_split_items<POSE, RAWF>(rp, st, pts, models, tags, model_count, slot_score, slot_inl, plan, totals);
+}
+
+constexpr int FIRST_THREADS = 256;
+constexpr int FIRST_PICK_MAX = 64;
+MDRP_GLOBAL __launch_bounds__(FIRST_THREADS) void k_first_pick(RunParams rp, const PairState *__restrict__ st, const int32_t *__restrict__ surv_count,
+                                                              const uint32_t *__restrict__ tags_in , int pick,
+                                                              uint32_t *__restrict__ tags_pick, int32_t *__restrict__ pick_count ,
+                                                              uint32_t *__restrict__ tags_rest, int32_t *__restrict__ rest_count ) {
+    const int pair = blockIdx.x, tid = threadIdx.x;
+    if (!st[pair].active) return;
+    __builtin_amdgcn_s_setprio(3);
+    __shared__ int s_hist[256];
+    __shared__ int s_key, s_need, s_prefix, s_first, s_np, s_nr;
+    const int cnt = surv_count[pair];
+    const size_t slot_base = (size_t)pair * rp.slot_stride;
+    const uint32_t *src = tags_in + slot_base;
+    s_hist[tid] = 0;
+    if (tid == 0) { s_first = 0x7FFFFFFF; s_np = 0; s_nr = 0; }
+    __syncthreads();
+    for (int i = tid; i < cnt; i += FIRST_THREADS) {
+        const uint32_t t = src[i];
+        atomicAdd(&s_hist[min(t >> 24, (uint32_t)PROBE_PTS)], 1);
+        atomicMin(&s_first, (int)(t & 0xFFFFFFu));
+    }
+    __syncthreads();
+    if (tid == 0) {
+        int key = -1, above = 0;
+        if (cnt > pick)
+            for (key = PROBE_PTS; key > 0 && above + s_hist[key] < pick; --key) above += s_hist[key];
+        s_key = key; s_need = pick - above; s_prefix = 0;
+    }
+    __syncthreads();
+    const int key_t = s_key;
+    for (int shift = 16; shift >= 0 && key_t >= 0; shift -= 8) {
+        s_hist[tid] = 0;
+        __syncthreads();
+        const int prefix = s_prefix;
+        for (int i = tid; i < cnt; i += FIRST_THREADS) {
+            const uint32_t t = src[i], slot = t & 0xFFFFFFu;
+            if ((int)min(t >> 24, (uint32_t)PROBE_PTS) == key_t && (int)(slot >> (shift + 8)) == prefix) atomicAdd(&s_hist[(slot >> shift) & 255u], 1);
+        }
+        __syncthreads();
+        if (tid == 0) {
+            int b = 0, acc = 0;
+            for (; b < 255 && acc + s_hist[b] < s_need; ++b) acc += s_hist[b];
+            s_need -= acc; s_prefix = (prefix << 8) | b;
+        }
+        __syncthreads();
+    }
+    const uint32_t slot_s = (uint32_t)s_prefix, first = (uint32_t)s_first;
+    uint32_t *dp = tags_pick + slot_base, *dr = tags_rest + slot_base;
+    for (int i = tid; i < cnt; i += FIRST_THREADS) {
+        const uint32_t t = src[i], slot = t & 0xFFFFFFu;
+        const int key = (int)min(t >> 24, (uint32_t)PROBE_PTS);
+        if (key > key_t || (key == key_t && slot <= slot_s) || slot == first) dp[atomicAdd(&s_np, 1)] = t;
+        else dr[atomicAdd(&s_nr, 1)] = t;
+    }
+    __syncthreads();
+    if (tid == 0) { pick_count[pair] = s_np; rest_count[2 * pair] = s_nr; }
+    __builtin_amdgcn_s_setprio(0);
+}
+
+template <bool POSE, bool RAWF = false>
+__global__ __launch_bounds__(SPLIT_THREADS, MDRP_SCORE_MINWAVES) void k_first_score(RunParams rp, const PairState *__restrict__ st, const double *__restrict__ pts,
+                                                               const Model *__restrict__ models, const uint32_t *__restrict__ tags,
+                                                               const int32_t *__restrict__ model_count, double *__restrict__ slot_score,
+                                                               int32_t *__restrict__ slot_inl, const int32_t *__restrict__ plan,
+                                                               const int32_t *__restrict__ totals) {
+    __builtin_amdgcn_s_setprio(3);
+    score_split_items<POSE, RAWF>(rp, st, pts, models, tags, model_count, slot_score, slot_inl, plan, totals);
+    __builtin_amdgcn_s_setprio(0);
+}
+
+MDRP_GLOBAL __launch_bounds__(FIRST_THREADS) void k_first_filter(RunParams rp, const PairState *__restrict__ st, const double *__restrict__ slot_score,
+                                                                const int32_t *__restrict__ slot_inl, const uint32_t *__restrict__ tags_pick,
+                                                                const int32_t *__restrict__ pick_count, const uint32_t *__restrict__ tags_rest,
+                                                                const int32_t *__restrict__ rest_count , uint32_t *__restrict__ tags_out,
+                                                                int32_t *__restrict__ surv_count, unsigned long long *__restrict__ evals) {
+    const int pair = blockIdx.x, tid = threadIdx.x;
+    const PairState &ps = st[pair];
+    if (!ps.active) return;
+    __builtin_amdgcn_s_setprio(3);
+    __shared__ int32_t s_iter[FIRST_PICK_MAX + 1], s_cnt[FIRST_PICK_MAX + 1];
+    __shared__ double s_score[FIRST_PICK_MAX + 1];
+    __shared__ int s_kept;
+    const int n = ps.n, np = min(pick_count[pair], FIRST_PICK_MAX + 1), nr = rest_count[2 * pair];
+    const double thr = ps.sq_thr;
+    const size_t slot_base = (size_t)pair * rp.slot_stride;
+    if (tid < np) {
+        const uint32_t slot = tags_pick[slot_base + tid] & 0xFFFFFFu;
+        s_iter[tid] = (int32_t)(slot / (uint32_t)rp.mps);
+        s_cnt[tid] = slot_inl[slot_base + slot];
+        s_score[tid] = slot_score[slot_base + slot];
+    }
+    if (tid == 0) s_kept = 0;
+    __syncthreads();
+    for (int i = tid; i < nr; i += FIRST_THREADS) {
+        const uint32_t t = tags_rest[slot_base + i], slot = t & 0xFFFFFFu;
+        const RecordBar bar = prefix_bar(s_iter, s_cnt, s_score, np, (int)(slot / (uint32_t)rp.mps));
+        if (!bar.retires(n, thr, cand_of_key((int)min(t >> 24, (uint32_t)PROBE_PTS), n))) tags_out[slot_base + atomicAdd(&s_kept, 1)] = t;
+    }
+    __syncthreads();
+    if (tid == 0) {
+        surv_count[pair] = s_kept;
+        if (evals) atomicAdd(evals, (unsigned long long)np * (unsigned long long)n);
+    }
+    __builtin_amdgcn_s_setprio(0);
 }
 
 template <int MPS = 4, int IPL = 1>
diff --git a/mdrp_amd/csrc/mdrp_schedule.h b/mdrp_amd/csrc/mdrp_schedule.h
--- a/mdrp_amd/csrc/mdrp_schedule.h
+++ b/mdrp_amd/csrc/mdrp_schedule.h
@@ -107,6 +107,22 @@
 inline int lo_lanes(int batch_call, int n_max) { return (batch_call >= 128 && n_max < 4096) ? 64 : 256; }
 inline int final_lanes(int batch_call) { return batch_call >= 4096 ? 64 : 256; }
 
+constexpr int FIRST_PICK = 48, FIRST_PICK_LIMIT = 64;
+inline int first_pick(int kind, int batch_call, int wave_max_pairs, int knob) {
+    if (kind > MDRP_VARYING_FOCAL || batch_call <= wave_max_pairs) return 0;
+    return knob < 0 ? FIRST_PICK : std::min(knob, FIRST_PICK_LIMIT);
+}
+
+constexpr size_t LDS_GRANULE = 2560;
+inline size_t solver_reservation(size_t lds_per_cu, int resident_per_simd, size_t keep_free) {
+    if (resident_per_simd <= 0 || keep_free >= lds_per_cu) return 0;
+    const size_t wgs = 4 * (size_t)resident_per_simd;
+    const size_t bytes = (lds_per_cu - keep_free) / wgs / LDS_GRANULE * LDS_GRANULE;
+    if (bytes == 0 || (wgs + 1) * bytes <= lds_per_cu) return 0;
+    return bytes;
+}
+constexpr int SOLVE_RESIDENT = 2;
+
 inline long long fuse_n_scale(int n_max) { return std::max(1, (n_max + 1999) / 2000); }
 inline int fuse_gate_us(int batch, int n_max) { return (int)std::min<long long>((50000 + 40ll * batch) * fuse_n_scale(n_max), 200000); }
 inline int fuse_wait_us(int batch, int n_max) { return (int)std::min<long long>((20000 + 4ll * batch) * fuse_n_scale(n_max), 100000); }
```
